# bark-simulator/planner-miqp

Measured on AMD Instinct MI355X. Metric: MIQP solves/sec to 1% gap, 2-agent x 20-step x 32-region, higher is better.
Workload: dtype f64

## Files before the change

include/miqp_gpu.h:

```cpp
#ifndef MIQP_GPU_H
#define MIQP_GPU_H

#include "miqp_types.h"

#ifdef __cplusplus
extern "C" {
#endif

typedef struct miqp_solver miqp_solver_t;

typedef struct miqp_solver_opts {
  int precision;
  int device;
  int nodes_per_round;
  int max_open_nodes;
  double gap_override;
  int verbose;
} miqp_solver_opts;

miqp_solver_t* miqp_solver_create(const miqp_solver_opts* opts);
void miqp_solver_destroy(miqp_solver_t* s);

int miqp_solver_set_params(miqp_solver_t* s, const miqp_model_params_c* p);

int miqp_solver_load_dat(miqp_solver_t* s, const char* path);

int miqp_solver_override_settings(miqp_solver_t* s, double max_solution_time, double relative_mip_gap_tolerance);

int miqp_solver_set_warmstart(miqp_solver_t* s, const miqp_raw_results_c* start, int warmstart_type);

int miqp_solver_solve(miqp_solver_t* s, double timestamp);

int miqp_solver_solve_batch(miqp_solver_t* const* solvers, int n, int* statuses);

int miqp_solver_solve_stream(miqp_solver_t* const* solvers, int n, int inflight, int* statuses);

int miqp_solver_solve_batch_multi(miqp_solver_t* const* solvers, int n, int gpus, int* statuses);

typedef int (*miqp_exchange_fn)(void* user, int op, void* buf, int count, int root);
int miqp_solver_solve_split(miqp_solver_t* s, double timestamp, int world, int rank, miqp_exchange_fn exchange, void* user);

int miqp_comm_unique_id(char* out128);
int miqp_comm_init(int world, int rank, const char* id128, int device);
int miqp_comm_finalize(void);
int miqp_solver_solve_split_rccl(miqp_solver_t* s, double timestamp);
int miqp_comm_selftest(miqp_exchange_fn exchange, void* user, int world, int rank);

int miqp_solver_split_roots(const miqp_solver_t* s, int world, int rank, int* root_of_pair, int* index, int* value, int cap, int* nroots_out, int* ncombos_out);

int miqp_solver_raw_sizes(const miqp_solver_t* s, int* out4);
int miqp_solver_lift_tables(const miqp_solver_t* s, double* out, int cap);

int miqp_solver_get_results(const miqp_solver_t* s, miqp_raw_results_c* out);

int miqp_solver_materialize_results(miqp_solver_t* const* solvers, int n, int threads);

int miqp_solver_get_properties(const miqp_solver_t* s, miqp_solution_properties_c* out);

int miqp_solver_get_dims(const miqp_solver_t* s, int* out6);

int miqp_solver_export_lp(const miqp_solver_t* s, const char* path);

int miqp_solver_write_dat(const miqp_solver_t* s, const char* path);

int miqp_solver_write_solution(const miqp_solver_t* s, const char* path);

int miqp_solver_write_mst(const miqp_solver_t* s, const char* path);

int miqp_solver_read_mst(miqp_solver_t* s, const char* path);

int miqp_solver_solve_fixed(miqp_solver_t* s, const miqp_raw_results_c* fixed, miqp_raw_results_c* out,
                            double* objective, int* iterations);

int miqp_solver_last_timing(const miqp_solver_t* s, double* out6);

int miqp_solver_last_active_set(const miqp_solver_t* s, double* out8);

int miqp_solver_last_fixed_route(const miqp_solver_t* s);

int miqp_solver_solve_fixed_batch(miqp_solver_t* s, const miqp_raw_results_c* const* fixed, int n, miqp_fixed_result_c* out, int* best);

int miqp_solver_fixed_batch_record(miqp_solver_t* s, int k, miqp_raw_results_c* out);

int miqp_gpu_fixed_result_size(void);
int miqp_gpu_fixed_batch_chunk(void);

int miqp_solver_set_pool(miqp_solver_t* s, int capacity);
int miqp_solver_pool_count(const miqp_solver_t* s);
int miqp_solver_pool_found(const miqp_solver_t* s, double* obj, int cap);
int miqp_solver_pool_solve(miqp_solver_t* s, miqp_fixed_result_c* out, int cap);
int miqp_solver_pool_record(miqp_solver_t* s, int k, miqp_raw_results_c* out);
int miqp_gpu_pool_max(void);

int miqp_solver_set_pool_filter(miqp_solver_t* s, int families);
int miqp_gpu_pool_signature(int cars, int steps, int obstacles, int families, const signed char* decisions, signed char* out, int len);
int miqp_solver_pool_signature(const miqp_solver_t* s, const miqp_raw_results_c* rec, int families, signed char* out, int cap);
int miqp_solver_pool_found_decisions(const miqp_solver_t* s, int k, signed char* out, int cap);

int miqp_solver_solve_fixed_multi(miqp_solver_t* const* solvers, int n, const miqp_raw_results_c* const* fixed, const int* first, miqp_fixed_result_c* out, int* best);
int miqp_solver_pool_solve_multi(miqp_solver_t* const* solvers, int n, miqp_fixed_result_c* out, int cap, int* counts);

int miqp_gpu_has_active_set(int num_cars, int num_steps);

int miqp_solver_launch_plan(const miqp_solver_t* s, int bc, int overlap, int par, const int* cls_n3, int cus, double free_gb, int flags, int* out, int cap);

int miqp_solver_last_setup(const miqp_solver_t* s, double* out3);

int miqp_solver_last_admission(const miqp_solver_t* s, double* out1);

const char* miqp_solver_last_error(const miqp_solver_t* s);


int miqp_fraction_parameters(int nr_regions, float max_velocity_fitting, double* out);
int miqp_fitting_polynomial_parameters(int nr_regions, float max_velocity_fitting, float min_velocity_fitting, double* out);
int miqp_mean_angles(const double* fraction_parameters, int nr_regions, double* out);
int miqp_limits_per_region(const double* fraction_parameters, int nr_regions, float long_min, float long_max, float lat_min, float lat_max,
                           double* min_x, double* max_x, double* min_y, double* max_y);
int miqp_calculate_region_idx(const double* fraction_parameters, int nr_regions, float vx, float vy, int* out);
int miqp_reserve_neighbor_regions(int* row, int nr_regions, int expansions);
int miqp_calculate_possible_regions(const double* fraction_parameters, int nr_regions, const double* theta_ref, int n, int* flags);
int miqp_reference_trajectory(const double* ref_xy, int n_ref, const double* state5, double dt, int num_points, double line_interp_inc, double vel_desired,
                              double delta_s_desired, double acc_lat_max, int vel_curve_dep, double* out);
int miqp_update_car(const double* settings12, const double* fraction_parameters, const double* initial_state6, const double* ref_xy, int n_ref, double desired_velocity,
                    double delta_s_desired, double timestep, int track_reference_positions, int is_ego, int num_cars, double* ref4N, int* possible_region, double* weights8);
int miqp_calculate_warmstart(const miqp_raw_results_c* last, miqp_raw_results_c* out, double ts, double minimum_region_change_speed);
int miqp_plan(miqp_solver_t* s, miqp_model_params_c* p, int* initial_region, int* possible_region, const miqp_raw_results_c* warmstart,
              int warmstart_type, double timestamp, int* status_out);

int miqp_initial_pose_check(const miqp_model_params_c* p);
int miqp_select_environment(const double* pieces_xy, const int* piece_off, int n_pieces, const double* traj_xy, const int* traj_off, int n_traj, int* selected);
int miqp_obstacle_intersects_environment(const double* pieces_xy, const int* piece_off, int n_pieces, const double* obstacle_xy, int n_steps, int is_static);
int miqp_bark_trajectory(const miqp_raw_results_c* results, int car, double start_time, double ts, double min_speed, double* out_rows5);
int miqp_obstacles_roi(double x, double y, double theta, double behind_distance, double front_distance, double side_distance, double* roi_xy);
int miqp_obstacle_intersects_environment_roi(const double* pieces_xy, const int* piece_off, int n_pieces, const double* obstacle_xy, int n_steps, int is_static, const double* roi_xy);
int miqp_environment_warmstart(const miqp_raw_results_c* last, miqp_raw_results_c* out, const int* ids_old, int n_old, const int* ids_new, int n_new);

int miqp_solver_certify(miqp_solver_t* s, const miqp_raw_results_c* candidate, miqp_certificate_c* out);
int miqp_solver_certify_batch(miqp_solver_t* const* solvers, int n, miqp_certificate_c* out);
int miqp_gpu_certificate_size(void);
int miqp_gpu_certify_last_timing(double* out4);

const char* miqp_gpu_version(void);

#ifdef __cplusplus
}
#endif
#endif
```

planner_miqp_amd/csrc/as_onchip.hip:

```cpp
namespace miqp {

#ifdef MIQP_PROFILE
#define ASP_T(var) const long long var = clock64()
#define ASP_ACC(k, t0, t1) asp_[k] += (unsigned long long)((t1) - (t0))
#else
#define ASP_T(var)
#define ASP_ACC(k, t0, t1)
#endif
constexpr int AS_MAXSTEP = 220;
constexpr double AS_VTOL = 1.0e-8;
constexpr double AS_DEP = 1.0e-8;
constexpr int AS_MT = 64;
constexpr int AS_MSTR = AS_MT * (AS_MT + 1) / 2;

__host__ __device__ constexpr bool as_shape_ok(int C, int N) { return (C == 1 || C == 2) && N >= 1 && N <= 2 * OC_NSL; }

template <int C> __device__ inline int as_col(int pq) { return C == 2 ? ((pq & 3) << 2) | (pq >> 2) : ((pq & 1) << 2) | (pq >> 1); }
template <int C> __device__ inline int as_pcol(int q) { return C == 2 ? ((q & 3) << 2) | (q >> 2) : ((q & 3) << 1) | (q >> 2); }
template <int C> struct AsDecode {
  static constexpr bool LANE_BOUNDS = true, ROW_IDENTITY = true, MARKS = true;
  static __device__ int col(int l) { return as_col<C>(oc_pcol<C, true>(l)); }
};

template <int C, int NSL, int GCAP = miqp::OC_GCAP>
__global__ void __launch_bounds__(64, (GCAP > 128 ? 1 : 2)) as_onchip_kernel(DevBuf B) {
  static_assert(C == 1 || C == 2, "a stage of 16 columns holds the chains of up to two cars");
  constexpr bool CM = true;
  constexpr bool BIG = GCAP > 128;
  constexpr int OC_GCAP = GCAP, OC_GSLOTS = OC_GCAP / 64, OC_GCOEF = oc_gcoef_of(OC_GCAP);
  constexpr int NX = 6 * C, NZ = 8 * C, NCH = 2 * C;
  const Layout& Y = B.Y;
  const int tid = threadIdx.x, lg = tid >> 4, lc = tid & 15;
  const int par = lg >> 1, side = lg & 1;
  const double bsgn = side ? -1.0 : 1.0;
  WAVE_DUMP(BIG ? 1 : 4);
  const int* const clist = BIG && B.cls_take ? B.cls_list + (size_t)(B.cls_take - 1) * B.batch_cap : nullptr;
  const int nbatch = clist ? (B.cls_count[B.cls_take - 1] < B.batch_cap ? B.cls_count[B.cls_take - 1] : B.batch_cap) : (*B.batch_count < B.batch_cap ? *B.batch_count : B.batch_cap);
  const int N = Y.N, NSLOT = Y.NSLOT;
  extern __shared__ double lds[];
  char* const L0 = (char*)lds;
  const OcLds LL = oc_lds_layout(N, Y.fixlen, OC_GCAP, !BIG);
  double* const Z = (double*)(L0 + LL.z);
  double* const scr = (double*)(L0 + LL.u);
  double* const V = (double*)(L0 + LL.u);
  unsigned long long* const bkey = (unsigned long long*)(L0 + LL.r);
  const int SPAN = LL.gmeta - LL.u;
  double* const kref = (double*)(L0 + LL.u + SPAN - N * 32);
  double* const kff = kref - N * 4;
  double* const KS = kff - N * 16;
  const int STG_CAP = (SPAN - N * 192) / 8;
  uint4* const gmeta = (uint4*)(L0 + LL.gmeta);
  double* const gcoef = (double*)(L0 + LL.gcoef);
  double* const grhs = (double*)(L0 + LL.grhs);
  double* const Wd = (double*)(L0 + LL.wd);
  int* const sstart = (int*)(L0 + LL.sstart);
  unsigned short* const cand = (unsigned short*)(L0 + LL.cand);
  signed char* const fix = (signed char*)(L0 + LL.fix);
  __shared__ int sh_node;
  __shared__ unsigned long long sh_stat[32];
  if (tid < 32) sh_stat[tid] = 0ull;
  const unsigned long long lt = (1ull << tid) - 1ull;

  const int chunk = B.as_chunk > 0 ? B.as_chunk : 1;
  int run_next = 0, run_end = 0;
  const int quota = BIG ? 0 : B.as_quota; int handed = 0;
#ifdef MIQP_PROFILE
  const unsigned long long wv_c0 = __builtin_amdgcn_s_memtime(), wv_r0 = __builtin_amdgcn_s_memrealtime();
  unsigned long long wv_first = 0; int wv_nodes = 0;
  if (!BIG && tid == 0) wv_first = atomicMin(&B.prof[120], wv_r0);
#endif
  for (;;) {
    __syncthreads();
    if (run_next >= run_end) {
      if (quota > 0 && handed >= quota) break;
      ++handed;
      if (tid == 0) sh_node = atomicAdd(B.work_counter, chunk);
      __syncthreads();
      run_next = __builtin_amdgcn_readfirstlane(sh_node); run_end = run_next + chunk;
      if (run_next >= nbatch) break;
    }
    const int slot_ = run_next++;
    if (slot_ >= nbatch) { run_next = run_end; continue; }
    const int node = clist ? __builtin_amdgcn_readfirstlane(clist[slot_]) : slot_;
    {
      const int cls = B.batch_large ? (int)B.batch_large[node] : (is_probe_word(B.batch_depth[node]) ? 1 : 0);
      if (cls != (BIG ? 1 : 0)) continue;
    }
    WAVE_DUMP_NODE();
    const int inst = __builtin_amdgcn_readfirstlane(B.batch_inst[node]);
    const double* D = B.inst_d + (size_t)inst * Y.dstride;
    const int* T = B.inst_i + (size_t)inst * Y.istride;
    const double ts = D[Y.d_glob + 7];
    const double aqs = 2.0 * D[Y.d_misc + 0];
    const double iaq = aqs > 0.0 ? 1.0 / aqs : 0.0;
    {
      const signed char* src = B.pool_fix + (size_t)B.batch_node[node] * Y.fixlen;
      for (int k = tid; k < Y.fixlen; k += 64) fix[k] = src[k];
      if (tid < 16) Wd[tid] = tid < NZ ? D[Y.d_wd + oc_lcol<C, CM>(as_pcol<C>(tid))] : 0.0;
      for (int k = tid; k < N * 32; k += 64) bkey[k] = ~0ull;
      for (int k = tid; k <= N + 1; k += 64) sstart[k] = 0;
    }
    __syncthreads();
    const double* Rf = D + Y.d_ref;
    double cutoff = 1e300;
    {
      const double inc0 = fmin(inc_from_key(*(volatile unsigned long long*)&B.inc_key[inst]), B.inc_ext[inst]);
      const double gap_ = is_probe_word(B.batch_depth[node]) ? 0.0 : B.inst_gap[inst];
      if (B.use_cutoff && inc0 < 1e300) cutoff = inc0 - gap_ * (1e-10 + fabs(inc0)) - B.inst_const[inst];
    }

#ifdef MIQP_PROFILE
    unsigned long long asp_[12] = {0, 0, 0, 0, 0, 0, 0, 0, 0, 0, 0, 0};
#endif
    ASP_T(ta0);
#define OC_DECODE_POLICY AsDecode<C>
#include "oc_decode_body.inc"
#undef OC_DECODE_POLICY
    if (overflow) {
      if (B.batch_A) B.batch_A[(size_t)node * 64 + tid] = 0xFFFFu;
      if (tid == 0) {
        if (B.ring_M) B.batch_Mtag[node] = 0ull;
        B.batch_ok[node] = 5; B.pool_big[B.batch_node[node]] |= (BIG ? 2 : 1); if (B.stats) { atomicAdd(&B.stats[3], 1ull); atomicAdd(&B.stats[8 + (ngen >= 512 ? 15 : ngen / 32)], 1ull); }
      }
      continue;
    }
    const int NM = sstart[N + 1];
    OC_WAVE_SYNC();

    ASP_T(ta1); ASP_ACC(0, ta0, ta1);
#ifdef MIQP_PROFILE
    asp_[9] += (unsigned long long)(ocd_t_sparse - ta0); asp_[11] += (unsigned long long)(ta1 - ocd_t_rows);
#endif
    double brhs[NSL];
    unsigned int bact = 0u, binA = 0u, ginA = 0u;
#pragma unroll
    for (int k = 0; k < NSL; ++k) {
      const int i = 2 * k + par;
      brhs[k] = 1e300;
      if (i < N && lc < NZ) {
        const unsigned long long key = bkey[(i * 2 + side) * 16 + lc];
        if (key != ~0ull) { brhs[k] = key2d(key); bact |= 1u << k; }
      }
    }
    OC_WAVE_SYNC();

    const double h1 = ts, h2 = 0.5 * ts * ts, h3 = ts * ts * ts / 6.0;
    const double* const tb = D + Y.d_astab;
    if constexpr (C == 2) {
      for (int k = tid; k < N * 16; k += 64) KS[k] = tb[k];
      for (int k = tid; k < N * 4; k += 64) kref[k] = tb[N * 16 + k];
    } else {
      for (int k = tid; k < N * 8; k += 64) KS[(k >> 3) * 16 + (k & 7)] = tb[k];
      for (int k = tid; k < N * 2; k += 64) kref[(k >> 1) * 4 + (k & 1)] = tb[N * 8 + k];
    }
    OC_WAVE_SYNC();
    typedef double d2_t __attribute__((ext_vector_type(2)));
    auto subst = [&](const bool fromx0, const int itop, const int iend, double* const out) {
      for (int k = tid; k < (N - 1) * 4; k += 64) if ((k >> 2) > itop) kff[k] = fromx0 ? kref[k] : 0.0;
      if (tid < NCH) {
        const int ch = tid;
        double p0 = 0.0, p1 = 0.0, p2 = 0.0;
        int i0 = itop;
        if (itop >= N - 1) { const d2_t a = *(const d2_t*)(V + (N - 1) * 16 + 4 * ch); p0 = a[0]; p1 = a[1]; p2 = V[(N - 1) * 16 + 4 * ch + 2]; i0 = N - 2; }
        if (i0 >= 0) {
          d2_t va = *(const d2_t*)(V + i0 * 16 + 4 * ch), vb = *(const d2_t*)(V + i0 * 16 + 4 * ch + 2);
          d2_t ka = *(const d2_t*)(KS + (i0 * 4 + ch) * 4), kb = *(const d2_t*)(KS + (i0 * 4 + ch) * 4 + 2);
          double kr = fromx0 ? kref[i0 * 4 + ch] : 0.0;
          for (int i = i0; i >= 0; --i) {
            const int j = i > 0 ? i - 1 : 0;
            const d2_t nva = *(const d2_t*)(V + j * 16 + 4 * ch), nvb = *(const d2_t*)(V + j * 16 + 4 * ch + 2);
            const d2_t nka = *(const d2_t*)(KS + (j * 4 + ch) * 4), nkb = *(const d2_t*)(KS + (j * 4 + ch) * 4 + 2);
            const double nkr = fromx0 ? kref[j * 4 + ch] : 0.0;
            const double su = vb[1] + h3 * p0 + h2 * p1 + h1 * p2;
            const double sx0 = va[0] + p0, sx1 = va[1] + h1 * p0 + p1, sx2 = vb[0] + h2 * p0 + h1 * p1 + p2;
            kff[i * 4 + ch] = fma(su, kb[1], kr);
            p0 = sx0 - ka[0] * su; p1 = sx1 - ka[1] * su; p2 = sx2 - kb[0] * su;
            va = nva; vb = nvb; ka = nka; kb = nkb; kr = nkr;
          }
        }
      }
      OC_WAVE_SYNC();
      if (tid < NCH) {
        const int ch = tid;
        double x0 = 0.0, x1 = 0.0, x2 = 0.0;
        if (fromx0) { const int c = ch >> 1, s = ch & 1; x0 = D[Y.d_x0 + 6 * c + 3 * s]; x1 = D[Y.d_x0 + 6 * c + 3 * s + 1]; x2 = D[Y.d_x0 + 6 * c + 3 * s + 2]; }
        const int ie = iend < N - 1 ? iend : N - 2;
        d2_t ka = *(const d2_t*)(KS + ch * 4), kb = *(const d2_t*)(KS + ch * 4 + 2);
        double kf = kff[ch];
        for (int i = 0; i <= ie; ++i) {
          const int j = i < N - 2 ? i + 1 : N - 2;
          const d2_t nka = *(const d2_t*)(KS + (j * 4 + ch) * 4), nkb = *(const d2_t*)(KS + (j * 4 + ch) * 4 + 2);
          const double nkf = kff[j * 4 + ch];
          const double u = -kf - (ka[0] * x0 + ka[1] * x1 + kb[0] * x2);
          d2_t oa, ob; oa[0] = x0; oa[1] = x1; ob[0] = x2; ob[1] = u;
          *(d2_t*)(out + i * 16 + 4 * ch) = oa; *(d2_t*)(out + i * 16 + 4 * ch + 2) = ob;
          const double n0 = x0 + h1 * x1 + h2 * x2 + h3 * u, n1 = x1 + h1 * x2 + h2 * u, n2 = x2 + h1 * u;
          x0 = n0; x1 = n1; x2 = n2;
          ka = nka; kb = nkb; kf = nkf;
        }
        if (iend >= N - 1 || ie == N - 2) { d2_t oa, ob; oa[0] = x0; oa[1] = x1; ob[0] = x2; ob[1] = 0.0; *(d2_t*)(out + (ie + 1) * 16 + 4 * ch) = oa; *(d2_t*)(out + (ie + 1) * 16 + 4 * ch + 2) = ob; }
      }
      OC_WAVE_SYNC();
    };
    auto row_dot = [&](int id, const double* vec) -> double {
      if (id < 1024) return (((id >> 4) & 1) ? -1.0 : 1.0) * vec[(id >> 5) * 16 + (id & 15)];
      const uint4 m4 = gmeta[id - 1024];
      const int off = (int)(m4.z & 0xFFFFu), nn = (int)((m4.z >> 16) & 7u), i = (int)((m4.z >> 20) & 0x7FFu);
      double a = 0.0;
#pragma unroll
      for (int k = 0; k < 6; ++k) if (k < nn) a += gcoef[off + k] * vec[i * 16 + ((m4.w >> (4 * k)) & 15u)];
      return a;
    };
    auto row_soft = [&](int id) -> bool { return id >= 1024 && (gmeta[id - 1024].z & 0x80000000u) != 0u; };
    auto zeroV = [&]() { for (int k = tid; k < N * 16; k += 64) V[k] = 0.0; OC_WAVE_SYNC(); };
    auto objective = [&]() -> double {
      double o = 0.0;
      for (int k = tid; k < N * 16; k += 64) { const int q = k & 15; if (q < NZ) { const double d = Z[k] - Rf[(k >> 4) * NZ + oc_lcol<C, CM>(as_pcol<C>(q))]; o += Wd[q] * d * d; } }
      return wave_sum(o);
    };

    int arow = -1, astage = -1; double alam = 0.0, arhs = 0.0;
    double M[64];
#pragma unroll
    for (int b = 0; b < 64; ++b) M[b] = 0.0;
    unsigned long long used = 0ull;
    auto rank1 = [&](const double u, const double alpha, const unsigned long long mask) {
#pragma unroll
      for (int g8 = 0; g8 < 8; ++g8) {
        if ((mask >> (8 * g8)) & 0xFFull) {
#pragma unroll
          for (int j = 0; j < 8; ++j) { const int b = 8 * g8 + j; M[b] = fma(u * readlane_d(u, b), alpha, M[b]); }
        }
      }
    };
    auto refresh = [&]() {
      zeroV();
      const double FX = 274877906944.0, IFX = 1.0 / 274877906944.0;
      if (arow >= 0 && alam != 0.0) {
        if (arow < 1024) atomicAdd((unsigned long long*)&V[(arow >> 5) * 16 + (arow & 15)], (unsigned long long)(long long)__double2ll_rn((((arow >> 4) & 1) ? -alam : alam) * FX));
        else {
          const uint4 m4 = gmeta[arow - 1024];
          const int off = (int)(m4.z & 0xFFFFu), nn = (int)((m4.z >> 16) & 7u), i = (int)((m4.z >> 20) & 0x7FFu);
#pragma unroll
          for (int k = 0; k < 6; ++k) if (k < nn) atomicAdd((unsigned long long*)&V[i * 16 + ((m4.w >> (4 * k)) & 15u)], (unsigned long long)(long long)__double2ll_rn(gcoef[off + k] * alam * FX));
        }
      }
      OC_WAVE_SYNC();
      for (int k = tid; k < N * 16; k += 64) V[k] = (double)(long long)__double_as_longlong(V[k]) * IFX;
      const int amax = (int)wave_max((double)astage);
      OC_WAVE_SYNC();
      subst(true, amax, N - 1, Z);
    };
    if constexpr (C == 2) { for (int k = tid; k < N * 16; k += 64) Z[k] = tb[N * 20 + k]; }
    else { for (int k = tid; k < N * 16; k += 64) Z[k] = (k & 15) < NZ ? tb[N * 10 + (k >> 4) * NZ + (k & 15)] : 0.0; }
    OC_WAVE_SYNC();
    ASP_T(ta2); ASP_ACC(1, ta1, ta2);
    int steps = 0, ndrop = 0, ok = 1, nwarm = 0, nfast = 0, ncold = 0;
    bool infeas = false, fail = false;
    int why = 0;
    if (B.pool_A && (B.batch_depth[node] >> 6) >= 1 && B.batch_node[node] < B.z_cap) {
      const int rec = B.batch_node[node];
      const unsigned int pa = B.pool_A[(size_t)rec * 64 + tid];
      int cid = -1;
      int ownl = 0;
      if (pa < 1024u) ownl = (int)((((pa >> 5) & 1u) * 2u + ((pa >> 4) & 1u)) << 4 | (pa & 15u));
      const unsigned int ob = (unsigned int)__shfl((int)bact, ownl);
      if (pa < 1024u) { if ((ob >> (pa >> 6)) & 1u) cid = (int)pa; }
      else if (pa != 0xFFFFu) {
        const int pc = (int)pa - 1024;
        int lo = 0, hi = NM;
        while (lo < hi) { const int mid = (lo + hi) >> 1; if ((int)cand[mid] < pc) lo = mid + 1; else hi = mid; }
        if (lo < NM && (int)cand[lo] == pc) cid = 1024 + lo;
      }
      const unsigned long long u0p = __ballot(pa != 0xFFFFu);
      const unsigned long long u0 = __ballot(cid >= 0);
      if (u0) {
        arow = cid;
        astage = cid < 0 ? -1 : (cid < 1024 ? (cid >> 5) : (int)((gmeta[cid - 1024].z >> 20) & 0x7FFu));
        int nmp = 0; unsigned long long moff = 0ull;
        if (B.ring_M) {
          const unsigned long long tg = B.pool_Mtag[rec];
          const unsigned long long c_ = tg >> 8;
          if (tg != 0ull && *(volatile unsigned long long*)B.ring_head - c_ < B.ring_doubles - B.ring_margin) { nmp = (int)(tg & 255ull); moff = c_ % B.ring_doubles; }
        }
// ... 161 lines not shown
        const int r = q * 64 + tid;
        if (r < NM && !((ginA >> q) & 1u)) { const double rh_ = grhs[r]; const double v = row_dot(1024 + r, Z) - rh_; if (v > bv) { bv = v; brh = rh_; bid = 1024 + r; } }
      }
      const double vmax = wave_max(bv);
      if (!(vmax > AS_VTOL)) break;
      if (steps >= AS_MAXSTEP || used == ~0ull || !(vmax < 1e290)) { fail = true; why = used == ~0ull ? 1 : 2; break; }
      const int src = __builtin_amdgcn_readfirstlane(__ffsll((long long)__ballot(bv == vmax)) - 1);
      const int pid = __builtin_amdgcn_readlane(bid, src);
      const bool psoft = row_soft(pid);
      const double prhs = readlane_d(brh, src);
      ASP_T(tb1); ASP_ACC(2, tb0, tb1);
      zeroV();
      if (pid < 1024) { if (tid == 0) V[(pid >> 5) * 16 + (pid & 15)] = ((pid >> 4) & 1) ? -1.0 : 1.0; }
      else {
        const uint4 m4 = gmeta[pid - 1024];
        const int off = (int)(m4.z & 0xFFFFu), nn = (int)((m4.z >> 16) & 7u), i = (int)((m4.z >> 20) & 0x7FFu);
        if (tid < nn) V[i * 16 + ((m4.w >> (4 * tid)) & 15u)] = gcoef[off + tid];
      }
      const int pstage = pid < 1024 ? (pid >> 5) : (int)((gmeta[pid - 1024].z >> 20) & 0x7FFu);
      const int amax_ = (int)wave_max((double)astage);
      OC_WAVE_SYNC();
      subst(false, pstage, amax_ > pstage ? amax_ : pstage, V);
      ASP_T(tb2); ASP_ACC(3, tb1, tb2);
      double q = arow >= 0 ? -row_dot(arow, V) : 0.0;
      const double Spp = -row_dot(pid, V) + (psoft ? iaq : 0.0);
      double vp = vmax, lp = 0.0;
      steps++;
      ASP_T(tb3); ASP_ACC(4, tb2, tb3);
      for (;;) {
        double r = 0.0;
#pragma unroll
        for (int g8 = 0; g8 < 8; ++g8) {
          if ((used >> (8 * g8)) & 0xFFull) {
#pragma unroll
            for (int j = 0; j < 8; ++j) { const int b = 8 * g8 + j; r = fma(M[b], readlane_d(q, b), r); }
          }
        }
        if (arow < 0) r = 0.0;
        const double curv = Spp - wave_sum(q * r);
        const double ratio = (arow >= 0 && r > 1e-13) ? alam / r : 1e300;
        const double td = wave_min(ratio);
        const int kd = td < 1e299 ? __builtin_amdgcn_readfirstlane(__ffsll((long long)__ballot(ratio == td)) - 1) : -1;
        if (!(curv == curv) || !(Spp > 0.0)) { fail = true; why = 3; break; }
        const bool dep = !(curv > AS_DEP * Spp);
        double t; bool full;
        if (dep) { if (kd < 0) { infeas = true; break; } t = td; full = false; }
        else { const double tp = vp / curv; if (tp <= td) { t = tp; full = true; } else { t = td; full = false; } }
        if (arow >= 0) { alam = fma(-t, r, alam); if (alam < 0.0) alam = 0.0; }
        lp += t;
        Dval += t * (vp - 0.5 * t * (dep ? 0.0 : curv));
        if (lp > RHO_EL) { infeas = true; break; }
        if (full) {
          const int s = __builtin_amdgcn_readfirstlane(__ffsll((long long)~used) - 1);
          double u = arow >= 0 ? r : 0.0;
          if (tid == s) u = -1.0;
          const unsigned long long nmask = used | (1ull << s);
          rank1(u, 1.0 / curv, nmask);
          if (tid == s) { arow = pid; alam = lp; astage = pstage; arhs = prhs; }
          used = nmask;
          if (pid < 1024) { if (tid == ((((pid >> 5) & 1) * 2 + ((pid >> 4) & 1)) << 4 | (pid & 15))) binA |= 1u << (pid >> 6); }
          else { const int rr_ = pid - 1024; if (tid == (rr_ & 63)) ginA |= 1u << (rr_ >> 6); }
          break;
        }
        vp -= t * (dep ? 0.0 : curv);
        const int idk = __builtin_amdgcn_readlane(arow, kd);
        if (idk < 1024) { if (tid == ((((idk >> 5) & 1) * 2 + ((idk >> 4) & 1)) << 4 | (idk & 15))) binA &= ~(1u << (idk >> 6)); }
        else { const int rr_ = idk - 1024; if (tid == (rr_ & 63)) ginA &= ~(1u << (rr_ >> 6)); }
        double m = 0.0;
#pragma unroll
        for (int b = 0; b < 64; ++b) m = (b == kd) ? M[b] : m;
        const double mkk = readlane_d(m, kd);
        if (!(mkk > 0.0)) { fail = true; why = 4; break; }
        rank1(m, -1.0 / mkk, used);
#pragma unroll
        for (int b = 0; b < 64; ++b) if (b == kd || tid == kd) M[b] = 0.0;
        if (tid == kd) { arow = -1; astage = -1; alam = 0.0; q = 0.0; }
        used &= ~(1ull << kd);
        ndrop++; steps++;
        if (steps >= AS_MAXSTEP) { fail = true; why = 2; break; }
      }
      ASP_T(tb4); ASP_ACC(5, tb3, tb4);
      if (infeas || fail) break;
      refresh();
      ASP_T(tb5); ASP_ACC(6, tb4, tb5);
      if (Dval - 1e-9 * fabs(Dval) > cutoff + 1e-9 * fabs(cutoff)) { ok = 2; break; }
    }
    ASP_T(tc0);
    double viol = 0.0, scost = 0.0, lres = 0.0;
    if (!fail && !infeas && ok == 1) {
#pragma unroll
      for (int k = 0; k < NSL; ++k) { const int i = 2 * k + par; if ((bact >> k) & 1u) viol = fmax(viol, bsgn * Z[i * 16 + lc] - brhs[k]); }
#pragma unroll
      for (int q = 0; q < OC_GSLOTS; ++q) { const int r = q * 64 + tid; if (r < NM && !(gmeta[r].z & 0x80000000u)) viol = fmax(viol, row_dot(1024 + r, Z) - grhs[r]); }
      if (arow >= 0) {
        const bool sf = arow >= 1024 && row_soft(arow);
        const double res = row_dot(arow, Z) - arhs - (sf ? alam * iaq : 0.0);
        if (sf) { scost = 0.5 * alam * alam * iaq; viol = fmax(viol, res); }
        lres = alam * res;
      }
      viol = wave_max(viol); scost = wave_sum(scost);
      lres = fabs(wave_sum(lres));
    } else if (infeas) viol = 1.0;
    if (!fail && !infeas && ok == 1 && !(viol <= 5.0e-7)) { fail = true; why = 5; }
    if (BIG && infeas && B.as_probe_first && B.pump_max > 0 && is_probe_word(B.batch_depth[node]) && (cutoff > 1e299 || B.pump_inc)) fail = true;
    if (fail) {
      if (B.batch_A) B.batch_A[(size_t)node * 64 + tid] = 0xFFFFu;
      if (B.ring_M && tid == 0) B.batch_Mtag[node] = 0ull;
      if (tid == 0) { B.batch_ok[node] = 5; B.pool_big[B.batch_node[node]] |= 4; if (B.as_stats) { sh_stat[2] += 1ull; sh_stat[10 + (why < 6 ? why : 5)] += 1ull; } }
      continue;
    }
    const double obj = (infeas || ok == 2) ? Dval : objective() + scost;
    double* Zo = B.batch_Z + (size_t)node * N * NZ;
    for (int k = tid; k < N * 16; k += 64) { const int q = k & 15; if (q < NZ) Zo[(k >> 4) * NZ + oc_lcol<C, CM>(as_pcol<C>(q))] = Z[k]; }
    if (B.batch_A) {
      unsigned short enc = 0xFFFFu;
      if (!fail && !infeas && ok == 1 && arow >= 0) enc = arow < 1024 ? (unsigned short)arow : (unsigned short)(1024 + (int)cand[arow - 1024]);
      B.batch_A[(size_t)node * 64 + tid] = enc;
    }
    if (B.ring_M) {
      const int n_ = __popcll(used);
      unsigned long long tg_ = 0ull;
      OC_WAVE_SYNC();
      if (!fail && !infeas && ok == 1 && n_ >= 1 && n_ <= AS_MT && n_ * (n_ + 1) * 4 <= LL.total) {
        double* const stg = (double*)L0;
        const int ra = __popcll(used & lt);
#pragma unroll
        for (int b8 = 0; b8 < 64; ++b8) {
          if ((used >> b8) & 1ull) {
            const int rb = __popcll(used & ((1ull << b8) - 1ull));
            if (arow >= 0 && ra >= rb) stg[ra * (ra + 1) / 2 + rb] = M[b8];
          }
        }
        const int len = n_ * (n_ + 1) / 2;
        unsigned long long cnt_ = 0ull;
        if (tid == 0) cnt_ = atomicAdd(B.ring_head, (unsigned long long)len);
        cnt_ = ((unsigned long long)(unsigned int)__builtin_amdgcn_readfirstlane((int)(cnt_ >> 32)) << 32) | (unsigned int)__builtin_amdgcn_readfirstlane((int)cnt_);
        tg_ = (cnt_ << 8) | (unsigned long long)n_;
        OC_WAVE_SYNC();
        const unsigned long long o_ = cnt_ % B.ring_doubles, rd_ = B.ring_doubles;
        for (int k = tid; k < len; k += 64) { unsigned long long q_ = o_ + (unsigned long long)k; if (q_ >= rd_) q_ -= rd_; B.ring_M[q_] = stg[k]; }
      }
      if (tid == 0) B.batch_Mtag[node] = tg_;
    }
    if (tid == 0) {
      B.batch_obj[node] = obj; B.batch_viol[node] = viol; B.batch_ok[node] = ok;
      B.batch_bound[node] = lres + 1e-9 * (1.0 + fabs(obj));
      B.batch_it[node] = steps;
      atomicAdd((unsigned long long*)&B.inst_nodes[inst], 1ull);
      atomicAdd((unsigned long long*)&B.inst_iters[inst], (unsigned long long)steps);
#ifdef MIQP_PROFILE
      ++wv_nodes;
      { const long long tc1 = clock64(); asp_[7] += (unsigned long long)(tc1 - tc0);
        for (int q_ = 0; q_ < 9; ++q_) atomicAdd(&B.prof[80 + q_], asp_[q_]);
        atomicAdd(&B.prof[92], asp_[9]); atomicAdd(&B.prof[93], asp_[11]);
        atomicAdd(&B.prof[90], 1ull); atomicAdd(&B.prof[91], (unsigned long long)steps); }
#endif
      if (B.as_stats) {
        sh_stat[0] += 1ull; sh_stat[1] += (unsigned long long)steps; sh_stat[3] += (unsigned long long)ndrop;
        sh_stat[4] += infeas ? 1ull : 0ull; sh_stat[5] += ok == 2 ? 1ull : 0ull; sh_stat[6] += (unsigned long long)__popcll(used); sh_stat[7] += (unsigned long long)nwarm; sh_stat[8] += (unsigned long long)nfast; sh_stat[9] += (unsigned long long)ncold;
        if (BIG) { const int og_ = B.pool_origin ? (int)B.pool_origin[B.batch_node[node]] : 0; sh_stat[20] += 1ull; sh_stat[21] += (unsigned long long)steps; if (og_ == 14) { sh_stat[22] += 1ull; sh_stat[23] += (unsigned long long)steps; }
          sh_stat[24 + (ngen <= 64 ? 0 : ngen <= 96 ? 1 : ngen <= 128 ? 2 : ngen <= 192 ? 3 : 4)] += 1ull; if (is_probe_word(B.batch_depth[node]) && og_ != 14) sh_stat[29] += 1ull; }
      }
    }
  }
  __syncthreads();
  if (B.as_stats && tid < 32 && sh_stat[tid] != 0ull) atomicAdd(&B.as_stats[tid], sh_stat[tid]);
#ifdef MIQP_PROFILE
  if (!BIG && tid == 0) {
    const unsigned long long wv_c1 = __builtin_amdgcn_s_memtime(), wv_r1 = __builtin_amdgcn_s_memrealtime();
    atomicAdd(&B.prof[94], wv_c1 - wv_c0); atomicAdd(&B.prof[95], wv_r1 - wv_r0); atomicAdd(&B.prof[96], 1ull);
    atomicMin(&B.prof[122], wv_r1); atomicMax(&B.prof[121], wv_r1);
    const unsigned long long dl = wv_r0 > wv_first ? wv_r0 - wv_first : 0ull;
    const int hb = dl < 5000 ? 0 : dl < 20000 ? 1 : dl < 50000 ? 2 : dl < 100000 ? 3 : dl < 200000 ? 4 : dl < 400000 ? 5 : dl < 800000 ? 6 : 7;
    atomicAdd(&B.prof[128 + hb], 1ull);
    const int nb = wv_nodes == 0 ? 0 : wv_nodes <= 4 ? 1 : wv_nodes <= 16 ? 2 : wv_nodes <= 32 ? 3 : wv_nodes <= 64 ? 4 : 5;
    atomicAdd(&B.prof[136 + nb], 1ull);
    if (B.prof[125] == 300 && blockIdx.x < 4096) {
      unsigned int hw, xcc;
      asm volatile("s_getreg_b32 %0, hwreg(HW_REG_HW_ID)" : "=s"(hw));
      asm volatile("s_getreg_b32 %0, hwreg(HW_REG_XCC_ID)" : "=s"(xcc));
      unsigned long long* const w = B.prof + 160 + 4 * blockIdx.x;
      w[0] = wv_r0; w[1] = wv_r1; w[2] = ((unsigned long long)xcc << 32) | hw; w[3] = (unsigned long long)wv_nodes;
    }
  }
#endif
}

}
```

planner_miqp_amd/csrc/ipm_onchip.hip:

```cpp
#ifndef MIQP_PHI_BRANCH
#define MIQP_PHI_BRANCH 1
#endif
namespace miqp {

constexpr int OC_GSLOTS = OC_GCAP / 64;
#ifndef MIQP_OC_PF
#define MIQP_OC_PF 4
#endif
constexpr int OC_PF = MIQP_OC_PF;
#ifndef MIQP_OC_GRP
#define MIQP_OC_GRP 5
#endif
constexpr int OC_GRP = MIQP_OC_GRP;
constexpr int OC_NSL = 10;

#ifdef MIQP_PROFILE
#define OCP_T(var) const long long var = clock64()
#define OCP_ACC(k, t0, t1) ocp_[k] += (unsigned long long)((t1) - (t0))
#elif defined(MIQP_ISA_MARKS)
#define OCP_T(var) asm volatile("; OCMARK " #var)
#define OCP_ACC(k, t0, t1)
#else
#define OCP_T(var)
#define OCP_ACC(k, t0, t1)
#endif
__host__ __device__ inline int oc_gain_doubles(int N) { return N * 64; }

template <int C, bool CM> __device__ inline int oc_pcol(int l) { return (CM && l < 6 * C) ? 2 * C * (l % 3) + l / 3 : l; }
template <int C, bool CM> __device__ inline int oc_lcol(int p) { return (CM && p < 6 * C) ? 3 * (p % (2 * C)) + p / (2 * C) : p; }
template <int C, bool CM> struct IpmDecode {
  static constexpr bool LANE_BOUNDS = false, ROW_IDENTITY = false, MARKS = false;
  static __device__ int col(int l) { return oc_pcol<C, CM>(l); }
};
template <int CTRL> __device__ inline double dpp_shift0(double x) {
  int lo = __double2loint(x), hi = __double2hiint(x);
  lo = __builtin_amdgcn_update_dpp(0, lo, CTRL, 0xF, 0xF, true);
  hi = __builtin_amdgcn_update_dpp(0, hi, CTRL, 0xF, 0xF, true);
  return __hiloint2double(hi, lo);
}

__device__ inline int fresh_lane() {
  int l;
  asm volatile("v_mbcnt_lo_u32_b32 %0, -1, 0\n\tv_mbcnt_hi_u32_b32 %0, -1, %0" : "=v"(l));
  return l;
}

__device__ inline void row_weight(double s, double lam, double t, bool soft, double aq, double tau, double& w, double& lk) {
  const double il = frcp(lam);
  double zz, r2mu = 0.0;
  if (!soft) { const double mu = RHO_EL - lam, im = frcp(mu); zz = t * im; r2mu = (tau - t * mu) * im; }
  else zz = frcp(aq);
  w = frcp(s * il + zz);
  lk = lam + ((tau - s * lam) * il - r2mu) * w;
}

template <int C, int NSL, int ABL = 0, int GCAP = miqp::OC_GCAP>
__global__ void __launch_bounds__(64, (GCAP > 128 ? 1 : 2)) ipm_onchip_kernel(DevBuf B) {
  constexpr int OC_ABL = ABL;
  constexpr int OC_GCAP = GCAP, OC_GSLOTS = GCAP / 64, OC_GCOEF = oc_gcoef_of(GCAP);
  constexpr bool BIG = GCAP > 128;
  static_assert(GCAP % 64 == 0 && GCAP <= 512, "general rows: whole register slots per lane, flags of up to 8 slots");
  constexpr bool CM = C == 2 && !(ABL & 1024);
  static_assert(C <= 2, "one 16 x 16 tile per stage");
  constexpr int NX = 6 * C, NU = 2 * C, NZ = 8 * C;
  constexpr int KB = (NX + 3) / 4;
  constexpr int RU = NX / 4, GU0 = NX % 4;
  const Layout& Y = B.Y;
  const int tid = threadIdx.x, lg = tid >> 4, lc = tid & 15;
  const int par = lg >> 1, side = lg & 1;
  const double bsgn = side ? -1.0 : 1.0;
  WAVE_DUMP(2);
  const int* const clist = BIG && B.cls_take ? B.cls_list + (size_t)(B.cls_take - 1) * B.batch_cap : nullptr;
  const int nbatch = clist ? (B.cls_count[B.cls_take - 1] < B.batch_cap ? B.cls_count[B.cls_take - 1] : B.batch_cap) : BIG && B.ovf_mode == 1 ? *B.ovf_count : (*B.batch_count < B.batch_cap ? *B.batch_count : B.batch_cap);
  const int N = Y.N, NSLOT = Y.NSLOT;
  extern __shared__ double lds[];
  char* const L0 = (char*)lds;
  const OcLds LL = oc_lds_layout(N, Y.fixlen, GCAP);
  double* const Z = (double*)(L0 + LL.z);
  double* const Dg = (double*)(L0 + LL.u);
  double* const Gd = Dg + N * 16;
  double* const dZ = Dg;
  double* const scr = Dg;
  unsigned long long* const bkey = (unsigned long long*)(L0 + LL.r);
  double* const gswfs = (double*)(L0 + LL.r);
#ifndef MIQP_KL0_PACK
#define MIQP_KL0_PACK 1
#endif
  constexpr int GS = (CM && MIQP_KL0_PACK) ? 1 : 2;
  constexpr int KL0N = OC_KL0 + (GS == 1 ? OC_GCAP / 64 : 0);
  double* const KL0 = gswfs + GS * OC_GCAP;
  uint4* const gmeta = (uint4*)(L0 + LL.gmeta);
  double* const gcoef = (double*)(L0 + LL.gcoef);
  double* const grhs = (double*)(L0 + LL.grhs);
  double* const Wd = (double*)(L0 + LL.wd);
  int* const sstart = (int*)(L0 + LL.sstart);
  unsigned short* const cand = (unsigned short*)(L0 + LL.cand);
  signed char* const fix = (signed char*)(L0 + LL.fix);
  double* const KG = B.kgain + (size_t)blockIdx.x * oc_gain_doubles(N);
  const double* KGs;
  { const unsigned long long a = (unsigned long long)KG;
    KGs = (const double*)(((unsigned long long)(unsigned int)__builtin_amdgcn_readfirstlane((int)(a >> 32)) << 32) | (unsigned int)__builtin_amdgcn_readfirstlane((int)a)); }
  const bool gown = lg < NU && lc <= NX;
  __shared__ int sh_node;
  const unsigned long long lt = (1ull << tid) - 1ull;

  for (;;) {
    __syncthreads();
    if (tid == 0) sh_node = atomicAdd(B.work_counter, 1);
    __syncthreads();
    if (__builtin_amdgcn_readfirstlane(sh_node) >= nbatch) break;
    const int node = __builtin_amdgcn_readfirstlane(clist ? clist[sh_node] : BIG && B.ovf_mode == 1 ? B.ovf_list[sh_node] : sh_node);
    if ((BIG && B.ovf_mode == 2) || (!BIG && B.skip_probes)) {
      const bool marked = B.batch_large ? B.batch_large[node] != 0 : is_probe_word(B.batch_depth[node]);
      if (BIG ? !marked : marked) continue;
      if (BIG && B.as_split && B.batch_large[node] != 2) continue;
    }
    WAVE_DUMP_NODE();
    const int inst = __builtin_amdgcn_readfirstlane(B.batch_inst[node]);
    const double* D = B.inst_d + (size_t)inst * Y.dstride;
    const int* T = B.inst_i + (size_t)inst * Y.istride;
    const double ts = D[Y.d_glob + 7];
    const double aqs = 2.0 * D[Y.d_misc + 0];
    {
      const signed char* src = B.pool_fix + (size_t)B.batch_node[node] * Y.fixlen;
      for (int k = tid; k < Y.fixlen; k += 64) fix[k] = src[k];
      if (tid < 16) Wd[tid] = tid < NZ ? D[Y.d_wd + oc_lcol<C, CM>(tid)] : 0.0;
      for (int k = tid; k < N * 16; k += 64) Z[k] = 0.0;
      for (int k = tid; k < N * 32; k += 64) bkey[k] = ~0ull;
      for (int k = tid; k <= N + 1; k += 64) sstart[k] = 0;
    }
    const bool warm = B.ws_on == 2 || (B.ws_on && B.pool_Z && (B.batch_depth[node] >> 6) >= 1 && B.batch_node[node] < B.z_cap);
    __syncthreads();
    if (warm) {
      const double* zp = B.ws_on == 2 ? B.inc_Z + (size_t)inst * N * NZ : B.pool_Z + (size_t)B.batch_node[node] * N * NZ;
      for (int k = tid; k < N * 16; k += 64) { const int q = k & 15; if (q < NZ) Z[k] = zp[(k >> 4) * NZ + oc_lcol<C, CM>(q)]; }
      OC_WAVE_SYNC();
    } else {
    if (tid < NX) Z[tid] = D[Y.d_x0 + oc_lcol<C, CM>(tid)];
    OC_WAVE_SYNC();
    for (int i = 0; i + 1 < N; ++i) {
      if (tid < NX) {
        double acc = 0;
        if (CM) { const int k = tid / (2 * C); acc = Z[i * 16 + tid]; if (k < 2) acc += ts * Z[i * 16 + tid + 2 * C]; if (k < 1) acc += 0.5 * ts * ts * Z[i * 16 + tid + 4 * C]; }
        else for (int q = 3 * (tid / 3); q < 3 * (tid / 3) + 3; ++q) acc += ab_entry<C>(tid, q, ts) * Z[i * 16 + q];
        Z[(i + 1) * 16 + tid] = acc;
      }
      OC_WAVE_SYNC();
    }
    }
    const double* Rf = D + Y.d_ref;
    const double cutoff = node_cutoff(B, inst, node);
#ifdef MIQP_PROFILE
    unsigned long long ocp_[12] = {0, 0, 0, 0, 0, 0, 0, 0, 0, 0, 0, 0};
#endif
    OCP_T(tp_d0);
    double abr[KB];
#pragma unroll
    for (int kb = 0; kb < KB; ++kb) abr[kb] = (!CM && 4 * kb + lg < NX && lc < NZ) ? ab_entry<C>(4 * kb + lg, lc, ts) : 0.0;

#define OC_DECODE_POLICY IpmDecode<C, CM>
#include "oc_decode_body.inc"
#undef OC_DECODE_POLICY
    if (overflow && !BIG && B.bounce) {
      if (tid == 0) { B.batch_ok[node] = 5; B.pool_big[B.batch_node[node]] |= 1; if (B.stats) { atomicAdd(&B.stats[3], 1ull); atomicAdd(&B.stats[8 + (ngen >= 512 ? 15 : ngen / 32)], 1ull); } }
      continue;
    }
    if (overflow && BIG && B.as_split) {
      if (tid == 0) { B.batch_ok[node] = 5; B.pool_big[B.batch_node[node]] |= 2; }
      continue;
    }
    if (overflow) {
      if (tid == 0) { const int q = atomicAdd(BIG ? B.ovf2_count : B.ovf_count, 1); (BIG ? B.ovf2_list : B.ovf_list)[q] = node; if (B.stats && !BIG) { atomicAdd(&B.stats[3], 1ull); atomicAdd(&B.stats[8 + (ngen >= 512 ? 15 : ngen / 32)], 1ull); if (ngen >= 480) { atomicMax(&B.stats[5], (unsigned long long)ngen); atomicAdd(&B.stats[6], (unsigned long long)ngen); atomicAdd(&B.stats[7], 1ull); } } }
      continue;
    }
    const int NM = sstart[N + 1];
    OC_WAVE_SYNC();
    if (tid == 0) { int a = 0; for (int i = 0; i <= N; ++i) { const int n = sstart[i]; a += n; sstart[i] = a; } }
    OC_WAVE_SYNC();

    double bs[NSL], bl[NSL], bt[NSL];
    unsigned int bact = 0u;
    double csum = 0.0, tsum = 0.0; int cnt = 0;
#pragma unroll
    for (int k = 0; k < NSL; ++k) {
// ... 527 lines not shown
```

planner_miqp_amd/csrc/miqp_gpu.hip:

```cpp
#include <hip/hip_runtime.h>
#include <dlfcn.h>

#include <algorithm>
#include <chrono>
#include <cmath>
#include <cstdio>
#include <cstdlib>
#include <cstring>
#include <map>
#include <memory>
#include <atomic>
#include <mutex>
#include <string>
#include <thread>
#include <vector>

#include "../../include/miqp_gpu.h"
#include "kernels.hip"
#include "wire_formats.hpp"
#include "planner_core.hpp"
#include "lp_export.hpp"

__attribute__((constructor)) static void miqp_gpu_hw_queues() { setenv("GPU_MAX_HW_QUEUES", "8", 0); }

// ... 1272 lines not shown
}
bool take_polished(const DevCtx& X, miqp_solver_t* const* S, int n, const HostTables& H, const Polished& P, Results& R) {
  const DevBuf& B = X.B; const Layout& Y = X.Y;
  std::vector<double> h_pZ((size_t)n * Y.N * Y.nz);
  HIP_OK(hipMemcpy(h_pZ.data(), B.batch_Z, h_pZ.size() * 8, hipMemcpyDeviceToHost));
  for (int k = 0; k < n; ++k) {
    if (!(R.inc[k] < 1e299)) continue;
    if (P.viol[k] <= FEAS_TOL && (P.ok[k] || P.it[k] >= 10)) {
      int nign = 0; for (int q = 0; q < Y.C * Y.O * Y.N * 5; ++q) nign += R.fix[(size_t)k * Y.fixlen + Y.f_obs + q] >= Y.L;
      R.inc[k] = P.obj[k] + H.h_const[k] + nign * S[k]->inst.w_slack_obs;
      std::copy(h_pZ.begin() + (size_t)k * Y.N * Y.nz, h_pZ.begin() + (size_t)(k + 1) * Y.N * Y.nz, R.Z.begin() + (size_t)k * Y.N * Y.nz);
    }
  }
  return true;
}

bool split_broadcast(const SplitCtx* split, const SplitState& sp, Results& R) {
  std::vector<unsigned char> buf(8 + R.Z.size() * 8 + R.fix.size());
  unsigned long long w[2] = {R.inc[0] < 1e299 ? ((host_d2key(R.inc[0]) & ~0xFFFFFull) | (unsigned long long)split->rank) : ~0ull, ~0ull};
  if (split->fn(split->user, 0, w, 2, 0) != 0) { std::fprintf(stderr, "[miqp_gpu] incumbent exchange failed\n"); return false; }
  if (w[0] < 0xFFF0000000000000ull) {
    const int owner = (int)(w[0] & 0xFFFFFull);
    if (owner == split->rank) { std::memcpy(buf.data(), &R.inc[0], 8); std::memcpy(buf.data() + 8, R.Z.data(), R.Z.size() * 8); std::memcpy(buf.data() + 8 + R.Z.size() * 8, R.fix.data(), R.fix.size()); }
    if (split->fn(split->user, 1, buf.data(), (int)buf.size(), owner) != 0) { std::fprintf(stderr, "[miqp_gpu] solution broadcast failed\n"); return false; }
    std::memcpy(&R.inc[0], buf.data(), 8); std::memcpy(R.Z.data(), buf.data() + 8, R.Z.size() * 8); std::memcpy(R.fix.data(), buf.data() + 8 + R.Z.size() * 8, R.fix.size());
    R.lb[0] = std::min(sp.lb, R.inc[0]);
  }
  R.flags[0] = sp.finished ? 0 : 1; R.oc[0] = 0; R.dn[0] = 1;
  return true;
}

struct CallTimes { double t_setup = 0, t_ctx = 0, t_tables = 0, t_solve = 0, ms_ipm = 0, ms_std = 0; float ms_all = 0; bool ctx_built = false, std_timed = false; };

void report(miqp_solver_t* const* S, int* statuses, const Layout& Y, const HostTables& H, const Rounds& L, const Results& R, const CallTimes& T, bool split) {
  const int n = L.n;
  long long tot_iters = 0; for (int k = 0; k < n; ++k) tot_iters += R.iters[k];
  for (int k = 0; k < n; ++k) {
    miqp_solver* s = S[k];
    bool have = R.inc[k] < 1e299;
    bool unfinished = (R.flags[k] & 3) || R.oc[k] > 0 || !R.dn[k];
    if (!split && k >= L.next_q && !H.h_done[k]) {
      s->status = MIQP_STATUS_FAILED_SEG_FAULT; s->has_sol = false; s->props.objective = NAN; s->props.gap = NAN; s->props.best_bound = NAN; s->props.status = 0; s->props.time = 0.0;
      s->err = "the queue was abandoned before this instance was admitted";
      statuses[k] = s->status; continue;
    }
    s->props.time = L.t_done[k] >= 0 ? L.t_done[k] : std::max(0.0, T.t_solve - L.t_admit[k]);
    s->admit_s = L.t_admit[k];
    s->props.NrIterations = (int)std::min<long long>(R.iters[k], 2147483647LL); s->props.nodes = R.nodes[k];
    s->props.NrSolutionPool = R.ninc[k];
    s->timing[0] = T.ms_all * 1e-3; s->timing[1] = T.ms_ipm * 1e-3; s->timing[2] = (double)(L.nev / 2); s->timing[3] = (double)L.launched_nodes;
    s->timing[4] = (double)tot_iters; s->timing[5] = (double)R.rowiters;
    s->as_timing[0] = (double)R.as[0]; s->as_timing[1] = (double)R.as[1]; s->as_timing[2] = (double)R.as[2]; s->as_timing[3] = (double)R.as[3];
    s->as_timing[4] = (double)R.as[6]; s->as_timing[5] = (double)R.as[7]; s->as_timing[6] = T.ms_std * 1e-3; s->as_timing[7] = T.std_timed ? (double)(L.nev / 2) : 0.0;
    s->setup[0] = T.t_setup; s->setup[1] = T.t_ctx; s->setup[2] = T.ctx_built ? 1.0 : 0.0;
    s->err.clear();
    if (L.stalled[k] && unfinished) s->err = "retired without a proof: no progress for 64 branch-and-bound rounds (not a time-limit verdict)";
    if (have) {
      s->status = MIQP_STATUS_SUCCESS; s->has_sol = true;
      s->props.objective = R.inc[k];
      double lb = std::min(R.lb[k], R.inc[k]);
      const double lb_tol = R.inc[k] - H.h_gap[k] * std::fabs(R.inc[k]);
      lb = std::min(lb, lb_tol);
      s->props.best_bound = lb; s->props.gap = std::fabs(lb - R.inc[k]) / (1e-10 + std::fabs(R.inc[k]));
      if (lb == lb_tol && s->props.gap > H.h_gap[k]) s->props.gap = H.h_gap[k];
      s->props.status = unfinished ? MIQP_CPX_STAT_TIME_LIM_FEAS : (s->props.gap <= 1e-9 ? MIQP_CPX_STAT_OPTIMAL : MIQP_CPX_STAT_OPTIMAL_TOL);
      s->Z.assign(R.Z.begin() + (size_t)k * Y.N * Y.nz, R.Z.begin() + (size_t)(k + 1) * Y.N * Y.nz);
      s->comp.assign(R.fix.begin() + (size_t)k * Y.fixlen, R.fix.begin() + (size_t)(k + 1) * Y.fixlen);
    } else {
      s->status = unfinished ? (L.stalled[k] ? MIQP_STATUS_FAILED_SEG_FAULT : MIQP_STATUS_FAILED_TIMEOUT) : MIQP_STATUS_FAILED_NO_SOLUT;
      s->props.objective = NAN; s->props.gap = NAN; s->props.best_bound = R.lb[k];
      s->props.status = unfinished ? MIQP_CPX_STAT_TIME_LIM_INFEAS : MIQP_CPX_STAT_INFEASIBLE;
    }
    statuses[k] = s->status;
  }
  if (L.abandoned) std::fprintf(stderr, "[miqp_gpu] the round loop was abandoned with %d of %d instances never admitted: they report FAILED_SEG_FAULT, the call fails\n", n - L.next_q, n);
}

bool pool_prepare(DevCtx& X, miqp_solver_t* const* S, int n);
bool pool_read_back(const DevCtx& X, miqp_solver_t* const* S, int n, const Results& R);

bool solve_batch_impl(miqp_solver_t* const* S, int n, int* statuses, const SplitCtx* split = nullptr, int inflight = 0, int lane = 0, int lanes = 1) {
  for (int k = 0; k < n; ++k) { statuses[k] = MIQP_STATUS_FAILED_SEG_FAULT; if (S[k]) { S[k]->status = MIQP_STATUS_FAILED_SEG_FAULT; S[k]->has_sol = false; S[k]->rescache.reset(); S[k]->drop_pool(); } }
  if (split && n != 1) return false;
  BatchShape bs = batch_layout(S, n);
  if (!bs.ok) { for (int k = 0; k < n; ++k) { if (S[k]) S[k]->err = bs.err; statuses[k] = MIQP_STATUS_FAILED_SEG_FAULT; } std::fprintf(stderr, "[miqp_gpu] %s\n", bs.err.c_str()); return false; }
  const Layout& Y = bs.Y;
  const miqp_solver_opts& O0 = S[0]->opts;
  auto fail_all = [&](const char* why) { if (why) std::fprintf(stderr, "[miqp_gpu] %s\n", why); for (int k = 0; k < n; ++k) statuses[k] = MIQP_STATUS_FAILED_SEG_FAULT; return false; };
  for (int k = 1; k < n; ++k) if (S[k]->opts.device != O0.device) return fail_all("instances of one batch must name the same device (use miqp_solver_solve_batch_multi to span devices)");
  const double t_enter = wall_s();
  DevCtx* Xp = ctx_for_device(O0.device, lane);
  if (!Xp) return fail_all(nullptr);
  warn_ignored_switches();
  DevCtx& X = *Xp;
  std::lock_guard<std::mutex> ctx_lock(X.mu);
  if (hipSetDevice(X.device) != hipSuccess) return fail_all("hipSetDevice failed");
  const CallSwitches sw = read_call_switches();
  const CallShape sh = plan_call(Y, O0, n, inflight, lanes, split != nullptr, sw);
  const size_t l_ipm = ipm_lds_bytes(Y), l_eval = eval_lds_bytes(Y, sw.seq_kinds);
  CallTimes T;
  {
    bool setup_ok = ctx_prepare(X, Y, n, sh.NS, sh.open_cap, sh.npr, sh.MAXR, sh.clamp_open, lanes, &T.ctx_built);
    if (setup_ok && (l_ipm > 160 * 1024 || l_eval > 160 * 1024)) { std::fprintf(stderr, "[miqp_gpu] instance too large for LDS (%zu bytes)\n", l_ipm); setup_ok = false; }
    if (setup_ok && !set_kernel_lds(Y, l_ipm, l_eval)) setup_ok = false;
    if (setup_ok && !pool_prepare(X, S, n)) setup_ok = false;
    if (split) {
      unsigned long long w = setup_ok ? 1ull : 0ull;
      if (split->fn(split->user, 0, &w, 1, 0) != 0) return fail_all("set-up exchange failed");
      if (setup_ok && w == 0ull) return fail_all("another rank of the tree split failed its set-up");
    }
    if (!setup_ok) return fail_all(nullptr);
  }
  T.t_ctx = wall_s() - t_enter;
  HostTables H;
  prepare_instances(S, Y, sh, split, H);
  T.t_tables = wall_s() - t_enter - T.t_ctx;
  apply_call_switches(X, sh, sw, H.h_gap);
  if (!upload_and_reset(X, H, sh)) return fail_all(nullptr);

  Rounds L(X, sh, H, split, O0.verbose, l_eval);
  if (!L.run()) return fail_all(nullptr);
  T.t_setup = L.t0 - t_enter;
  if (sw.dump_open && !dump_open_list(X, sw.dump_open, L.rounds, sh.NS, H.h_const[0])) return fail_all(nullptr);

  Polished P;
  if (!polish(X, n, P, T.ms_all)) return fail_all(nullptr);
#ifdef MIQP_PROFILE
  if (!print_profile(X)) return fail_all(nullptr);
#endif
  if (X.B.stats && !print_stats(X)) return fail_all(nullptr);
  if (process_switches().round_log) { std::fprintf(stderr, "[rounds]"); for (int v : L.round_bc) std::fprintf(stderr, " %d", v); std::fprintf(stderr, "\n"); }
  for (size_t e = 0; e + 1 < L.nev; e += 2) { float ms = 0; HIP_OK(hipEventElapsedTime(&ms, X.ipm_ev[e], X.ipm_ev[e + 1])); T.ms_ipm += ms; }
  T.std_timed = L.use_par;
  if (T.std_timed) for (size_t e = 0; e + 1 < L.nev; e += 2) { float ms = 0; if (hipEventElapsedTime(&ms, X.ipm_ev[e], X.std_ev[e / 2]) == hipSuccess) T.ms_std += ms; }
  T.t_solve = wall_s() - L.t0;

  Results R;
  if (!read_back(X, n, R) || !take_polished(X, S, n, H, P, R)) return fail_all(nullptr);
  if (X.pool.on && !pool_read_back(X, S, n, R)) return fail_all(nullptr);
  if (split && !split_broadcast(split, L.sp, R)) return fail_all(nullptr);
  report(S, statuses, Y, H, L, R, T, split != nullptr);
  for (int k = 0; k < n; ++k) if (!S[k]->has_sol) S[k]->drop_pool();
  if (sw.stats) std::fprintf(stderr, "[miqp_gpu stats] reachable-set diameter (L1) of instance 0: %.1f\n", H.D[Y.d_misc + 2]);
  if (sw.stats) std::fprintf(stderr, "[miqp_gpu stats] host: setup %.3f s (device context %.3f, instance tables and presolve %.3f, upload %.3f), rounds %.3f s (%d), results %.3f s\n", T.t_setup, T.t_ctx, T.t_tables, T.t_setup - T.t_ctx - T.t_tables, T.t_solve, L.rounds, wall_s() - L.t0 - T.t_solve);
  return !L.abandoned;
}

}

#include "certify.hip"
#include "fixed_batch.hip"
#include "solution_pool.hip"
#include "fixed_multi.hip"

extern "C" {

const char* miqp_gpu_version(void) { return "miqp_gpu 0.1 (gfx950)"; }

miqp_solver_t* miqp_solver_create(const miqp_solver_opts* opts) {
  miqp_solver* s = new miqp_solver();
  if (opts) s->opts = *opts; else { s->opts.precision = 12; s->opts.device = -1; s->opts.gap_override = -1; }
  if (s->opts.precision <= 0) s->opts.precision = 12;
  return s;
}

void miqp_solver_destroy(miqp_solver_t* s) { delete s; }

int miqp_solver_set_params(miqp_solver_t* s, const miqp_model_params_c* p) {
  if (!s || !p) return -1;
  s->has_inst = inst_from_params(p, s->opts.precision - 2, s->inst, s->err);
  s->rescache.reset(); s->drop_fixed_batch(); s->drop_pool();
  s->has_sol = false;
  if (!s->has_inst) std::fprintf(stderr, "[miqp_gpu] %s\n", s->err.c_str());
  return s->has_inst ? 0 : -2;
}

int miqp_solver_load_dat(miqp_solver_t* s, const char* path) {
  if (!s || !path) return -1;
  s->has_inst = inst_from_dat(path, s->inst, s->err);
  s->has_sol = false; s->rescache.reset(); s->drop_fixed_batch(); s->drop_pool();
  if (!s->has_inst) std::fprintf(stderr, "[miqp_gpu] %s\n", s->err.c_str());
  return s->has_inst ? 0 : -2;
}

int miqp_solver_override_settings(miqp_solver_t* s, double max_solution_time, double relative_mip_gap_tolerance) {
  if (!s || !s->has_inst) return -1;
  s->inst.tilim = max_solution_time; s->inst.gap = relative_mip_gap_tolerance;
  return 0;
}

int miqp_solver_get_dims(const miqp_solver_t* s, int* o) {
  if (!s || !s->has_inst) return -1;
  o[0] = s->inst.C; o[1] = s->inst.N; o[2] = s->inst.R; o[3] = s->inst.E; o[4] = s->inst.O; o[5] = s->inst.L;
  return 0;
}

int miqp_solver_set_warmstart(miqp_solver_t* s, const miqp_raw_results_c* start, int warmstart_type) {
  if (!s) return -1;
  if (warmstart_type == MIQP_WARMSTART_NONE || !start) { s->ws[0].reset(); s->ws[1].reset(); return 0; }
  const int slot = warmstart_type == MIQP_WARMSTART_LAST_SOLUTION ? 1 : 0;
  if (start->N < 2 || start->NrCars < 1 || start->NrRegions < 1 || start->NrEnvironments < 0 || start->NrObstacles < 0 || start->MaxLinesObstacles < 0 ||
      start->NrCarToCarCollisions != start->NrCars - 1) return -2;
  if (s->has_inst && !dims_match(*start, s->inst)) { s->ws[slot].reset(); return -3; }
  s->ws[slot].reset(new OwnedResults(start->NrCars, start->N, start->NrRegions, start->NrEnvironments, start->NrObstacles, start->MaxLinesObstacles));
  s->ws[slot]->copy_from(*start);
  return 0;
}

int miqp_solver_solve_batch(miqp_solver_t* const* solvers, int n, int* statuses) {
  if (!solvers || n < 1 || !statuses) return -1;
  return solve_batch_impl(solvers, n, statuses) ? 0 : -2;
}

int miqp_solver_solve_stream(miqp_solver_t* const* solvers, int n, int inflight, int* statuses) {
  if (!solvers || n < 1 || !statuses) return -1;
  int lanes = knob_int(KNOB_P("MIQP_LANES"), 1);
  if (lanes > 8) lanes = 8;
  while (lanes > 1 && (inflight <= 0 || inflight >= n || inflight / lanes < 128)) lanes--;
  if (lanes <= 1) return solve_batch_impl(solvers, n, statuses, nullptr, inflight) ? 0 : -2;
  for (int b = 0; b < n; ++b) { if (!solvers[b]) return -1; if (solvers[b]->opts.device != solvers[0]->opts.device) lanes = 1; }
  if (lanes <= 1) return solve_batch_impl(solvers, n, statuses, nullptr, inflight) ? 0 : -2;
  std::vector<std::vector<miqp_solver_t*>> sub(lanes); std::vector<std::vector<int>> st(lanes);
  for (int b = 0; b < n; ++b) sub[b % lanes].push_back(solvers[b]);
  std::vector<char> ok(lanes, 0);
  std::vector<std::thread> th;
  for (int l = 0; l < lanes; ++l) {
    st[l].assign(sub[l].size(), MIQP_STATUS_FAILED_SEG_FAULT);
    const int infl = (inflight + lanes - 1 - l) / lanes;
    th.emplace_back([&, l, infl] { ok[l] = solve_batch_impl(sub[l].data(), (int)sub[l].size(), st[l].data(), nullptr, infl, l, lanes) ? 1 : 0; });
  }
  for (auto& t : th) t.join();
  int rc = 0;
  for (int b = 0; b < n; ++b) statuses[b] = st[b % lanes][b / lanes];
  for (int l = 0; l < lanes; ++l) if (!ok[l]) rc = -2;
  return rc;
}

int miqp_solver_solve_batch_multi(miqp_solver_t* const* solvers, int n, int gpus, int* statuses) {
  if (!solvers || n < 1 || !statuses) return -1;
  int ndev = 0;
  if (hipGetDeviceCount(&ndev) != hipSuccess || ndev < 1) { std::fprintf(stderr, "[miqp_gpu] no HIP device: the solver has no CPU path\n"); for (int k = 0; k < n; ++k) statuses[k] = MIQP_STATUS_FAILED_SEG_FAULT; return -2; }
  if (gpus <= 0 || gpus > ndev) gpus = ndev;
  if (gpus > n) gpus = n;
  std::vector<std::vector<miqp_solver_t*>> shard(gpus); std::vector<std::vector<int>> st(gpus);
  for (int b = 0; b < n; ++b) { if (!solvers[b]) return -1; solvers[b]->opts.device = b % gpus; shard[b % gpus].push_back(solvers[b]); }
  std::vector<char> ok(gpus, 0);
  std::vector<std::thread> th;
  for (int g = 0; g < gpus; ++g) {
    st[g].assign(shard[g].size(), MIQP_STATUS_FAILED_SEG_FAULT);
    th.emplace_back([&, g] { ok[g] = solve_batch_impl(shard[g].data(), (int)shard[g].size(), st[g].data()) ? 1 : 0; });
  }
  for (auto& t : th) t.join();
  int rc = 0;
  for (int b = 0; b < n; ++b) statuses[b] = st[b % gpus][b / gpus];
  for (int g = 0; g < gpus; ++g) if (!ok[g]) rc = -2;
  return rc;
}

int miqp_solver_solve_split(miqp_solver_t* s, double timestamp, int world, int rank, miqp_exchange_fn exchange, void* user) {
  (void)timestamp;
  if (!s || !s->has_inst || world < 1 || rank < 0 || rank >= world || !exchange) return MIQP_STATUS_FAILED_SEG_FAULT;
  SplitCtx sc{world, rank, exchange, user};
  miqp_solver_t* one[1] = {s}; int st = MIQP_STATUS_FAILED_SEG_FAULT;
  if (!solve_batch_impl(one, 1, &st, &sc)) return MIQP_STATUS_FAILED_SEG_FAULT;
  return st;
}

int miqp_solver_split_roots(const miqp_solver_t* s, int world, int rank, int* root_of_pair, int* index, int* value, int cap, int* nroots_out, int* ncombos_out) {
  if (!s || !s->has_inst || world < 1 || rank < 0 || rank >= world) return -1;
  miqp_solver_t* one[1] = {const_cast<miqp_solver_t*>(s)};
  BatchShape bs = batch_layout(one, 1);
  if (!bs.ok) return -2;
  std::vector<double> D(bs.Y.dstride); std::vector<int> T(bs.Y.istride);
  compile_instance(s->inst, bs.Y, D.data(), T.data());
  std::vector<std::vector<std::pair<int, int>>> combos; split_roots(bs.Y, T.data(), combos, world);
  int np = 0, nr = 0;
  for (size_t q = 0; q < combos.size(); ++q) {
    if ((int)(q % (size_t)world) != rank) continue;
    for (auto& d : combos[q]) { if (np < cap) { if (root_of_pair) root_of_pair[np] = nr; if (index) index[np] = d.first; if (value) value[np] = d.second; } np++; }
    nr++;
  }
  if (nroots_out) *nroots_out = nr;
  if (ncombos_out) *ncombos_out = (int)combos.size();
  return np;
}

struct Id128 { char b[128]; };
namespace {
struct Rccl {
  void* lib = nullptr; void* comm = nullptr; int world = 0, rank = 0, device = -1; void* dbuf = nullptr; size_t dcap = 0; hipStream_t stream = nullptr;
  int (*GetUniqueId)(void*) = nullptr;
  int (*CommInitRank)(void**, int, Id128, int) = nullptr;
  int (*CommDestroy)(void*) = nullptr;
  int (*AllReduce)(const void*, void*, size_t, int, int, void*, hipStream_t) = nullptr;
  int (*Broadcast)(const void*, void*, size_t, int, int, void*, hipStream_t) = nullptr;
};
Rccl g_rccl; std::mutex g_rccl_mu;
bool rccl_load() {
  if (g_rccl.lib) return true;
  for (const char* nm : {"librccl.so.1", "librccl.so", "/opt/rocm/lib/librccl.so.1"}) { g_rccl.lib = dlopen(nm, RTLD_NOW | RTLD_LOCAL); if (g_rccl.lib) break; }
  if (!g_rccl.lib) { std::fprintf(stderr, "[miqp_gpu] librccl not found: %s\n", dlerror()); return false; }
  g_rccl.GetUniqueId = (int (*)(void*))dlsym(g_rccl.lib, "ncclGetUniqueId");
  g_rccl.CommInitRank = (int (*)(void**, int, Id128, int))dlsym(g_rccl.lib, "ncclCommInitRank");
  g_rccl.CommDestroy = (int (*)(void*))dlsym(g_rccl.lib, "ncclCommDestroy");
  g_rccl.AllReduce = (int (*)(const void*, void*, size_t, int, int, void*, hipStream_t))dlsym(g_rccl.lib, "ncclAllReduce");
  g_rccl.Broadcast = (int (*)(const void*, void*, size_t, int, int, void*, hipStream_t))dlsym(g_rccl.lib, "ncclBroadcast");
// ... 388 lines not shown
```

planner_miqp_amd/csrc/oc_decode.hip:

```cpp
namespace miqp {

constexpr int OC_GCAP = 128;
constexpr int OC_SCR = 32;
constexpr int OC_SSTR = 17;
constexpr int OC_KL0 = 6;

struct OcLds { int z, u, r, gmeta, gcoef, grhs, wd, sstart, cand, fix, total; };
constexpr int OC_GCAP_BIG = 320;
__host__ __device__ constexpr int oc_gcoef_of(int gcap) { return gcap == 128 ? 432 : gcap * 7 / 2; }
__host__ __device__ inline OcLds oc_lds_layout(int N, int fixlen, int OC_GCAP = miqp::OC_GCAP, bool as_std = false) {
  const int OC_GCOEF = oc_gcoef_of(OC_GCAP);
  OcLds L; int o = 0;
  L.z = o; o += N * 16 * 8;
  L.u = o; { int a = as_std ? N * 16 * 8 : N * 32 * 8, b = OC_SCR * OC_SSTR * 8; o += a > b ? a : b; }
  L.r = o; { int a = N * 32 * 8, b = as_std ? 0 : OC_GCAP * 16 + OC_KL0 * 64 * 8; o += a > b ? a : b; }
  L.gmeta = o; o += OC_GCAP * 16;
  L.gcoef = o; o += OC_GCOEF * 8;
  L.grhs = o; o += OC_GCAP * 8;
  L.wd = o; o += 16 * 8;
  L.sstart = o; o += ((N + 2) * 4 + 7) & ~7;
  L.cand = o; o += (OC_GCAP + 64) * 2;
  L.fix = o; o += (fixlen + 15) & ~15;
  L.total = (o + 15) & ~15;
  return L;
}

#define OC_WAVE_SYNC() do { __builtin_amdgcn_fence(__ATOMIC_RELEASE, "wavefront"); __builtin_amdgcn_wave_barrier(); __builtin_amdgcn_fence(__ATOMIC_ACQUIRE, "wavefront"); } while (0)

template <int C>
__device__ inline bool box_of_slot(const Layout& Y, const double* D, const int* T, const signed char* fix, int i, int slot, int& col, double& sgn, double& rhs) {
  if (slot >= C * Y.SC) return false;
  const int N = Y.N;
  const double* G = D + Y.d_glob;
  const int c = slot / Y.SC, rr = slot - c * Y.SC;
  const int code = i >= 1 ? (int)fix[Y.f_reg + c * N + i] : -1;
  const double* rt = code >= 0 ? D + Y.d_reg + (c * Y.P + (code >> 2)) * REGSZ : nullptr;
  if (rr < 7) {
    const double* Hc = (rt || rr < 3) ? D : region_hull(Y, D, T, fix, c, i);
    switch (rr) {
      case 0: col = 6 * c + 1; sgn = -1; rhs = -G[0]; break;
      case 1: col = 6 * c + 4; sgn = -1; rhs = -G[0]; break;
      case 2: col = 6 * c + 1; sgn = 1; rhs = G[1]; break;
      case 3: col = 6 * c + 2; sgn = 1; rhs = rt ? rt[12] : Hc[1]; break;
      case 4: col = 6 * c + 2; sgn = -1; rhs = -(rt ? rt[11] : Hc[0]); break;
      case 5: col = 6 * c + 5; sgn = 1; rhs = rt ? rt[14] : Hc[3]; break;
      default: col = 6 * c + 5; sgn = -1; rhs = -(rt ? rt[13] : Hc[2]); break;
    }
    return true;
  }
  if (rr < 11) {
    const int s = (rr - 7) >> 1; const bool up = ((rr - 7) & 1) == 0;
    double lo, hi;
    if (i == 0) { lo = D[Y.d_u0box + c * 4 + 2 * s]; hi = D[Y.d_u0box + c * 4 + 2 * s + 1]; }
    else if (rt) { lo = rt[15 + 2 * s]; hi = rt[16 + 2 * s]; }
    else { const double* Hc = region_hull(Y, D, T, fix, c, i); lo = Hc[4 + 2 * s]; hi = Hc[5 + 2 * s]; }
    col = 6 * C + 2 * c + s; sgn = up ? 1.0 : -1.0; rhs = up ? hi : -lo;
    return true;
  }
  if (rr < 16) {
    if (code < 0) return false;
    const int h = code & 3, k = rr - 11;
    if (h == 3) { col = 6 * c + (k < 2 ? 1 : 4); sgn = (k & 1) ? -1.0 : 1.0; rhs = G[6]; return true; }
    if (k == 2) {
      const int* hs = T + Y.i_hs + ((c * Y.P + (code >> 2)) * 2 + h) * 2;
      col = 6 * c + (hs[0] == 0 ? 1 : 4); sgn = -(double)hs[1]; rhs = -G[6];
      return true;
    }
    return false;
  }
  int q = rr - 16;
  const double* ed;
  if (q < 5 * Y.EL) {
    const int pt = q / Y.EL, k = q - pt * Y.EL;
    if (pt != 0) return false;
    const int e = Y.E == 1 ? 0 : (int)fix[Y.f_env + (c * N + i) * 5];
    ed = D + Y.d_env + (e * Y.EL + k) * 3;
  } else {
    q -= 5 * Y.EL;
    const int o = q / 5, pt = q - o * 5;
    if (pt != 0) return false;
    const int kk = (int)fix[Y.f_obs + ((c * Y.O + o) * N + i) * 5];
    ed = D + Y.d_obs + ((o * N + i) * Y.L + kk) * 3;
  }
  if (ed[1] == 0.0 && fabs(ed[0]) == 1.0) { col = 6 * c; sgn = ed[0]; rhs = ed[2]; return true; }
  if (ed[0] == 0.0 && fabs(ed[1]) == 1.0) { col = 6 * c + 3; sgn = ed[1]; rhs = ed[2]; return true; }
  return false;
}

template <int C>
__device__ inline bool slot_maybe(const Layout& Y, const signed char* fix, int i, int slot) {
  const int N = Y.N;
  if (slot < C * Y.SC) {
    const int c = slot / Y.SC, rr = slot - c * Y.SC;
    if (rr < 11) return true;
    if (i < 1) return false;
    const int code = (int)fix[Y.f_reg + c * N + i];
    if (rr < 16) return code >= 0 ? ((code & 3) != 3 || rr - 11 <= 3) : rr - 11 <= 1;
    int q = rr - 16;
    if (q < 5 * Y.EL) {
      if (Y.E < 1) return false;
      const int pt = q / Y.EL;
      const int e = Y.E == 1 ? 0 : (int)fix[Y.f_env + (c * N + i) * 5 + pt];
      return e >= 0 && (pt == 0 || code >= 0);
    }
    q -= 5 * Y.EL;
    const int o = q / 5, pt = q - o * 5;
    const int kk = (int)fix[Y.f_obs + ((c * Y.O + o) * N + i) * 5 + pt];
    return kk >= 0 && kk < Y.L && (pt == 0 || code >= 0);
  }
  if (C < 2 || i < 1) return false;
  const int q = slot - C * Y.SC;
  if (q < Y.NP * 8) { const int p = q >> 3, grp = (q & 7) >> 1; return (int)fix[Y.f_c2c + (p * N + i) * 4 + grp] >= 0; }
  const int q2 = q - Y.NP * 8, p = q2 >> 4, grp = (q2 >> 2) & 3, alt = q2 & 3;
  const int m = (int)fix[Y.f_c2n + (p * N + i) * 4 + grp];
  return m > 0 && ((m >> alt) & 1);
}

}
```

planner_miqp_amd/csrc/oc_decode_body.inc:

```
#ifdef MIQP_PROFILE
    long long ocd_t_sparse = 0, ocd_t_rows = 0;
#endif
    int ngen = 0;
    {
      unsigned long long* const bmp = (unsigned long long*)scr;
      const int nw = (N * NSLOT + 63) >> 6;
      unsigned short* const pre = (unsigned short*)(bmp + nw);
      for (int k = tid; k < nw; k += 64) bmp[k] = 0ull;
      OC_WAVE_SYNC();
      const int cls_off[8] = {0, 7, 11, 16, 16 + Y.EL, 16 + 5 * Y.EL, C * Y.SC, C * Y.SC + 8 * Y.NP};
      const int cls_cnt[8] = {7, 4, 5, Y.EL, 4 * Y.EL, 5 * Y.O, 8 * Y.NP, 16 * Y.NP};
      auto take = [&](int i, int slot) {
        if (decode_row<C, false>(Y, D, T, fix, i, slot, nullptr).active) {
          int col; double sg, rh;
          if (box_of_slot<C>(Y, D, T, fix, i, slot, col, sg, rh)) atomicMin(&bkey[(i * 2 + (sg < 0.0 ? 1 : 0)) * 16 + OC_DECODE_POLICY::col(col)], d2key(rh));
          else { const int pcode = i * NSLOT + slot; atomicOr(&bmp[pcode >> 6], 1ull << (pcode & 63)); }
        }
      };
      unsigned short* const plist = pre + ((nw + 1 + 3) & ~3);
      const int LCAP = (int)(((char*)(L0 + LL.r) - (char*)plist) / 2) - 64;
      int nlist = 0;
      auto flush = [&]() {
        OC_WAVE_SYNC();
        for (int j0 = 0; j0 < nlist; j0 += 64) if (j0 + tid < nlist) { const int pc = plist[j0 + tid]; const int i = pc / NSLOT; take(i, pc - i * NSLOT); }
        OC_WAVE_SYNC();
        nlist = 0;
      };
      if constexpr (OC_DECODE_POLICY::LANE_BOUNDS) {
        for (int e0 = 0; e0 < C * N; e0 += 64) {
          const int e = e0 + tid;
          if (e < C * N) {
            const int c = e / N, i = e - c * N;
            const double* G = D + Y.d_glob;
            const int code = i >= 1 ? (int)fix[Y.f_reg + c * N + i] : -1;
            const unsigned int skip = i >= 1 ? (unsigned int)T[Y.i_boxskip + c * N + i] : 0x7Fu;
            const double* rt = code >= 0 ? D + Y.d_reg + (c * Y.P + (code >> 2)) * REGSZ : nullptr;
            const double* Hc = (!rt && i >= 1) ? region_hull(Y, D, T, fix, c, i) : nullptr;
            auto put = [&](int col, bool neg, double rh) { atomicMin(&bkey[(i * 2 + (neg ? 1 : 0)) * 16 + OC_DECODE_POLICY::col(col)], d2key(rh)); };
            if (i >= 1) {
              const double a_lo_x = rt ? rt[11] : Hc[0], a_hi_x = rt ? rt[12] : Hc[1], a_lo_y = rt ? rt[13] : Hc[2], a_hi_y = rt ? rt[14] : Hc[3];
              if (!(skip & 1u)) put(6 * c + 1, true, -G[0]);
              if (!(skip & 2u)) put(6 * c + 4, true, -G[0]);
              if (!(skip & 4u)) put(6 * c + 1, false, G[1]);
              if (!(skip & 8u)) put(6 * c + 2, false, a_hi_x);
              if (!(skip & 16u)) put(6 * c + 2, true, -a_lo_x);
              if (!(skip & 32u)) put(6 * c + 5, false, a_hi_y);
              if (!(skip & 64u)) put(6 * c + 5, true, -a_lo_y);
            }
            if (i <= N - 2) {
#pragma unroll
              for (int s_ = 0; s_ < 2; ++s_) {
                double lo, hi;
                if (i == 0) { lo = D[Y.d_u0box + c * 4 + 2 * s_]; hi = D[Y.d_u0box + c * 4 + 2 * s_ + 1]; }
                else if (rt) { lo = rt[15 + 2 * s_]; hi = rt[16 + 2 * s_]; }
                else { lo = Hc[4 + 2 * s_]; hi = Hc[5 + 2 * s_]; }
                put(6 * C + 2 * c + s_, false, hi); put(6 * C + 2 * c + s_, true, -lo);
              }
            }
          }
        }
      }
#pragma unroll 1
      for (int cl = 0; cl < 8; ++cl) {
#ifdef MIQP_PROFILE
        if (OC_DECODE_POLICY::MARKS && cl == 2) ocd_t_sparse = clock64();
#endif
        const int cnt = cls_cnt[cl], off = cls_off[cl];
        const bool percar = cl < 6;
        const int per = percar ? C * cnt : cnt, total = N * per;
        for (int e0 = 0; e0 < total; e0 += 64) {
          const int e = e0 + tid;
          int i = 0, slot = 0; bool in = e < total;
          if (in) { i = e / per; const int rem = e - i * per; slot = percar ? (rem / cnt) * Y.SC + off + rem % cnt : off + rem; }
          if (cl < 2) {
            if constexpr (!OC_DECODE_POLICY::LANE_BOUNDS) { if (in) take(i, slot); }
            continue;
          }
          const bool cnd = in && slot_maybe<C>(Y, fix, i, slot);
          const unsigned long long mk = __ballot(cnd);
          if (cnd) plist[nlist + __popcll(mk & lt)] = (unsigned short)(i * NSLOT + slot);
          nlist += __popcll(mk);
          if (nlist > LCAP) flush();
        }
      }
      flush();
      if (tid == 0) { int a = 0; for (int k = 0; k < nw; ++k) { pre[k] = (unsigned short)(a < 65535 ? a : 65535); a += __popcll(bmp[k]); } pre[nw] = (unsigned short)(a < 65535 ? a : 65535); }
      OC_WAVE_SYNC();
      ngen = pre[nw];
      if (ngen <= OC_GCAP)
        for (int k = tid; k < nw; k += 64) {
          unsigned long long bits = bmp[k]; int pos = pre[k];
          while (bits) { const int b = __ffsll((long long)bits) - 1; cand[pos++] = (unsigned short)(k * 64 + b); bits &= bits - 1ull; }
        }
      OC_WAVE_SYNC();
    }
#ifdef MIQP_PROFILE
    if (OC_DECODE_POLICY::MARKS) ocd_t_rows = clock64();
#endif
    bool overflow = ngen > OC_GCAP;
    int ncoef = 0;
    for (int c0 = 0; c0 < ngen && !overflow; c0 += OC_SCR) {
      double* g = scr + (tid & (OC_SCR - 1)) * OC_SSTR;
      RowOut r; r.active = false; r.rhs = 0; r.aq = 0;
      int i = 0, nn = 0;
      const bool mine = tid < OC_SCR && c0 + tid < ngen;
      int slot_ = 0;
      if (mine) { const int pcode = cand[c0 + tid]; i = pcode / NSLOT; slot_ = pcode - i * NSLOT; r = decode_row<C, true>(Y, D, T, fix, i, slot_, g); }
      unsigned long long map = 0ull; unsigned int cols = 0u;
      double v6[6];
#pragma unroll
      for (int k = 0; k < 6; ++k) v6[k] = 0.0;
      if (mine) {
        for (int q = 0; q < NZ; ++q) {
          const double v = g[q];
          if (v != 0.0 && nn < 6) {
#pragma unroll
            for (int k = 0; k < 6; ++k) if (k == nn) v6[k] = v;
            const int pq = OC_DECODE_POLICY::col(q);
            map |= (unsigned long long)(nn + 1) << (4 * pq); cols |= (unsigned int)pq << (4 * nn); nn++;
          }
        }
      }
      const bool keep = mine && nn > 0;
      const unsigned long long mk = __ballot(keep);
      const unsigned long long b0 = __ballot(keep && (nn & 1)), b1 = __ballot(keep && (nn & 2)), b2 = __ballot(keep && (nn & 4));
      const int tot = __popcll(b0) + 2 * __popcll(b1) + 4 * __popcll(b2);
      if (ncoef + tot > OC_GCOEF) { overflow = true; break; }
      if (keep) {
        const int idx = sstart[N + 1] + __popcll(mk & lt);
        const int off = ncoef + __popcll(b0 & lt) + 2 * __popcll(b1 & lt) + 4 * __popcll(b2 & lt);
#pragma unroll
        for (int k = 0; k < 6; ++k) if (k < nn) gcoef[off + k] = v6[k];
        uint4 m4; m4.x = (unsigned int)map; m4.y = (unsigned int)(map >> 32);
        m4.z = (unsigned int)off | ((unsigned int)nn << 16) | ((unsigned int)i << 20) | (r.aq > 0.0 ? 0x80000000u : 0u); m4.w = cols;
        gmeta[idx] = m4; grhs[idx] = r.rhs;
        if constexpr (OC_DECODE_POLICY::ROW_IDENTITY) cand[idx] = (unsigned short)(i * NSLOT + slot_);
        else atomicAdd(&sstart[i + 1], 1);
      }
      OC_WAVE_SYNC();
      if (tid == 0) sstart[N + 1] += __popcll(mk);
      ncoef += tot;
      OC_WAVE_SYNC();
    }
```

planner_miqp_amd/csrc/solve_diag.hpp:

```cpp
#pragma once

inline void debug_sync(hipStream_t st, int round, const char* stage, int nodes = -1) {
  hipError_t e_ = hipStreamSynchronize(st);
  if (nodes >= 0) std::fprintf(stderr, "[dbg] round %d %s (%d nodes): %s\n", round, stage, nodes, hipGetErrorString(e_));
  else std::fprintf(stderr, "[dbg] round %d %s: %s\n", round, stage, hipGetErrorString(e_));
}

inline bool trace_selection(const DevCtx& X, int rounds, int bc) {
  const DevBuf& B = X.B;
  std::vector<double> sb(bc); std::vector<int> sd(bc); double io_ = 0; int md_ = 0;
  HIP_OK(hipMemcpy(sb.data(), B.batch_bound, (size_t)bc * 8, hipMemcpyDeviceToHost)); HIP_OK(hipMemcpy(sd.data(), B.batch_depth, (size_t)bc * 4, hipMemcpyDeviceToHost));
  HIP_OK(hipMemcpy(&io_, B.inc_obj, 8, hipMemcpyDeviceToHost)); HIP_OK(hipMemcpy(&md_, B.inst_mode, 4, hipMemcpyDeviceToHost));
  std::vector<int> ord(bc); for (int k = 0; k < bc; ++k) ord[k] = k;
  std::sort(ord.begin(), ord.end(), [&](int a, int b) { return sd[a] != sd[b] ? sd[a] > sd[b] : sb[a] < sb[b]; });
  std::fprintf(stderr, "[sel] r%d mode %d incumbent %a:", rounds, md_, io_);
  for (int k : ord) std::fprintf(stderr, " %d.%d/%a", sd[k] >> 6, sd[k] & 63, sb[k]);
  std::fprintf(stderr, "\n");
  return true;
}

inline bool trace_batch(const DevCtx& X, int rounds, int bc) {
  const DevBuf& B = X.B; hipStream_t st = X.stream;
  HIP_OK(hipStreamSynchronize(st));
  if (X.stream2) HIP_OK(hipStreamSynchronize(X.stream2));
  std::vector<int> hd(bc), hi(bc), hk(bc); std::vector<double> ho(bc), hb(bc), hv(bc);
  HIP_OK(hipMemcpy(hd.data(), B.batch_depth, bc * 4, hipMemcpyDeviceToHost)); HIP_OK(hipMemcpy(hi.data(), B.batch_it, bc * 4, hipMemcpyDeviceToHost));
  HIP_OK(hipMemcpy(hk.data(), B.batch_ok, bc * 4, hipMemcpyDeviceToHost)); HIP_OK(hipMemcpy(ho.data(), B.batch_obj, bc * 8, hipMemcpyDeviceToHost));
  HIP_OK(hipMemcpy(hb.data(), B.batch_bound, bc * 8, hipMemcpyDeviceToHost)); HIP_OK(hipMemcpy(hv.data(), B.batch_viol, bc * 8, hipMemcpyDeviceToHost));
  std::vector<int> ord(bc); for (int k = 0; k < bc; ++k) ord[k] = k;
  std::sort(ord.begin(), ord.end(), [&](int a, int b) { return hd[a] != hd[b] ? hd[a] < hd[b] : (ho[a] != ho[b] ? ho[a] < ho[b] : hi[a] < hi[b]); });
  { int oc_ = 0, fc_ = 0, tk_ = 0, dm_ = 0; double nt_ = 0;
    HIP_OK(hipMemcpy(&oc_, B.open_count, 4, hipMemcpyDeviceToHost)); if (B.far_cap > 0) HIP_OK(hipMemcpy(&fc_, B.far_count, 4, hipMemcpyDeviceToHost));
    HIP_OK(hipMemcpy(&nt_, B.near_thr, 8, hipMemcpyDeviceToHost)); HIP_OK(hipMemcpy(&tk_, B.slot_take, 4, hipMemcpyDeviceToHost)); HIP_OK(hipMemcpy(&dm_, B.slot_demand, 4, hipMemcpyDeviceToHost));
    std::fprintf(stderr, "[lists] r%d batch %d: near list after selection %d, far tier %d, near_thr %g, share of the next round %d, demand %d\n", rounds, bc, oc_, fc_, nt_, tk_, dm_); }
  for (int k : ord) std::fprintf(stderr, "[trace] r%d depth %d.%d ok %d it %d obj %a bound %a viol %.3e\n", rounds, hd[k] >> 6, hd[k] & 63, hk[k], hi[k], ho[k], hb[k], hv[k]);
  return true;
}

inline bool trace_launches(const DevCtx& X, int rounds, int bc, size_t nev) {
  const DevBuf& B = X.B; hipStream_t st = X.stream;
  HIP_OK(hipStreamSynchronize(st));
  float m1 = 0, m2 = 0; HIP_OK(hipEventElapsedTime(&m1, X.ipm_ev[nev], X.ev_mid)); HIP_OK(hipEventElapsedTime(&m2, X.ev_mid, X.ipm_ev[nev + 1]));
  int oc = 0; HIP_OK(hipMemcpy(&oc, B.ovf_count, 4, hipMemcpyDeviceToHost));
  std::vector<int> ol(std::max(oc, 1)), hit(bc), hdw(bc), hok(bc);
  if (oc > 0) HIP_OK(hipMemcpy(ol.data(), B.ovf_list, (size_t)oc * 4, hipMemcpyDeviceToHost));
  HIP_OK(hipMemcpy(hit.data(), B.batch_it, (size_t)bc * 4, hipMemcpyDeviceToHost)); HIP_OK(hipMemcpy(hdw.data(), B.batch_depth, (size_t)bc * 4, hipMemcpyDeviceToHost));
  HIP_OK(hipMemcpy(hok.data(), B.batch_ok, (size_t)bc * 4, hipMemcpyDeviceToHost));
  int np = 0, mxp = 0, mxo = 0, mxc = 0; long long sp = 0, so = 0, sc = 0;
  for (int q = 0; q < oc; ++q) { const int k = ol[q]; if ((hdw[k] & 63) == 63 && (hdw[k] >> 6) >= 1) { np++; sp += hit[k]; mxp = std::max(mxp, hit[k]); } else { so += hit[k]; mxo = std::max(mxo, hit[k]); } }
  std::vector<char> isov(bc, 0); for (int q = 0; q < oc; ++q) isov[ol[q]] = 1;
  for (int k = 0; k < bc; ++k) if (!isov[k]) { sc += hit[k]; mxc = std::max(mxc, hit[k]); }
  std::fprintf(stderr, "[launch] round %d nodes %d: on-chip %.2f ms (%d nodes, mean it %.1f, max %d); behind it %.2f ms: %d probes (mean it %.1f, max %d), %d others (mean it %.1f, max %d)\n",
               rounds, bc, m1, bc - oc, (double)sc / std::max(1, bc - oc), mxc, m2, np, (double)sp / std::max(1, np), mxp, oc - np, (double)so / std::max(1, oc - np), mxo);
  return true;
}

inline bool replay_batch(DevCtx& X, int bc) {
  static int replay = process_switches().replay;
  if (replay <= 0) return true;
  const DevBuf& B = X.B; hipStream_t st = X.stream; const Layout& Y = X.Y; (void)Y;
  hipEvent_t e0, e1; HIP_OK(hipEventCreate(&e0)); HIP_OK(hipEventCreate(&e1));
  HIP_OK(hipEventRecord(e0, st));
  for (int r = 0; r < replay; ++r) launch_ipm_batch(X, B, bc, st);
  HIP_OK(hipEventRecord(e1, st)); HIP_OK(hipStreamSynchronize(st));
  float ms = 0; HIP_OK(hipEventElapsedTime(&ms, e0, e1));
  std::vector<int> its(bc); HIP_OK(hipMemcpy(its.data(), B.batch_it, (size_t)bc * 4, hipMemcpyDeviceToHost));
  long long tot = 0; for (int v : its) tot += v;
  std::fprintf(stderr, "[miqp_gpu replay] %d nodes, %lld node-iterations: %.3f ms per pass, %.1f ns per node-iteration\n", bc, tot, ms / replay, 1e6 * ms / replay / (double)tot);
#ifdef MIQP_ABLATE
  if (X.oc_grid > 0 && Y.C == 2) {
    const size_t l_oc = (size_t)oc_lds_layout(Y.N, Y.fixlen).total;
    auto run = [&](auto kern, int mask) {
      HIP_OK(hipFuncSetAttribute((const void*)kern, hipFuncAttributeMaxDynamicSharedMemorySize, (int)l_oc));
      auto once = [&] { (void)hipMemsetAsync(B.work_counter, 0, 4, st); (void)hipMemsetAsync(B.ovf_count, 0, 4, st); hipLaunchKernelGGL(kern, dim3(std::min(bc, X.oc_grid)), dim3(64), l_oc, st, B); };
      once(); HIP_OK(hipEventRecord(e0, st)); for (int r = 0; r < 3; ++r) once(); HIP_OK(hipEventRecord(e1, st)); HIP_OK(hipStreamSynchronize(st));
      float m2 = 0; HIP_OK(hipEventElapsedTime(&m2, e0, e1));
      std::fprintf(stderr, "[miqp_gpu ablate] mask %4d: %.3f ms per pass of %d nodes x 15 iterations = %.1f ns per node-iteration\n", mask, m2 / 3, bc, 1e6 * m2 / 3 / (bc * 15.0));
      return true;
    };
    run(ipm_onchip_kernel<2, OC_NSL, 1>, 1); run(ipm_onchip_kernel<2, OC_NSL, 3>, 3); run(ipm_onchip_kernel<2, OC_NSL, 5>, 5); run(ipm_onchip_kernel<2, OC_NSL, 9>, 9);
    run(ipm_onchip_kernel<2, OC_NSL, 17>, 17); run(ipm_onchip_kernel<2, OC_NSL, 33>, 33); run(ipm_onchip_kernel<2, OC_NSL, 65>, 65); run(ipm_onchip_kernel<2, OC_NSL, 129>, 129);
    run(ipm_onchip_kernel<2, OC_NSL, 257>, 257); run(ipm_onchip_kernel<2, OC_NSL, 513>, 513); run(ipm_onchip_kernel<2, OC_NSL, 1023>, 1023);
    run(ipm_onchip_kernel<2, OC_NSL, 1025>, 1025);
    launch_ipm_batch(X, B, bc, st);
  }
#endif
  replay = 0;
  return true;
}

inline bool print_progress(const DevCtx& X, double t, int rounds, long long launched_nodes, double const0) {
  const DevBuf& B = X.B; hipStream_t st = X.stream;
  double lb0 = 0, io0 = 0; int oc0 = 0; unsigned long long k0 = 0;
  HIP_OK(hipMemcpyAsync(&lb0, B.lower_bound, 8, hipMemcpyDeviceToHost, st)); HIP_OK(hipMemcpyAsync(&io0, B.inc_obj, 8, hipMemcpyDeviceToHost, st));
  HIP_OK(hipMemcpyAsync(&oc0, B.open_count, 4, hipMemcpyDeviceToHost, st)); HIP_OK(hipMemcpyAsync(&k0, B.inc_key, 8, hipMemcpyDeviceToHost, st));
  int fc0 = 0; HIP_OK(hipMemcpyAsync(&fc0, B.far_count, 4, hipMemcpyDeviceToHost, st));
  HIP_OK(hipStreamSynchronize(st));
  std::fprintf(stderr, "[miqp_gpu] t %.2f s round %d nodes %lld: instance 0 bound %.4f incumbent %.4f open %d + %d\n", t, rounds, launched_nodes, lb0, k0 >= 0xFFF0000000000000ull ? INFINITY : io0 + const0, oc0, fc0);
  return true;
}

inline bool dump_open_list(const DevCtx& X, const char* dp, int rounds, int NS, double const0) {
  const DevBuf& B = X.B; const Layout& Y = X.Y; const int open_cap = X.open_cap;
  int oc0 = 0; HIP_OK(hipMemcpy(&oc0, B.open_count, 4, hipMemcpyDeviceToHost)); oc0 = std::min(oc0, open_cap);
  const size_t src = ((size_t)(rounds & 1) * NS + 0) * open_cap;
  std::vector<double> hb(oc0); std::vector<int> hn(oc0), hd(oc0);
  if (oc0 > 0) { HIP_OK(hipMemcpy(hb.data(), B.open_bound + src, (size_t)oc0 * 8, hipMemcpyDeviceToHost)); HIP_OK(hipMemcpy(hn.data(), B.open_node + src, (size_t)oc0 * 4, hipMemcpyDeviceToHost));
    HIP_OK(hipMemcpy(hd.data(), B.open_depth + src, (size_t)oc0 * 4, hipMemcpyDeviceToHost)); }
  std::vector<int> ord(oc0); for (int k = 0; k < oc0; ++k) ord[k] = k;
  std::sort(ord.begin(), ord.end(), [&](int x, int y) { return hb[x] < hb[y]; });
  if (FILE* f = std::fopen(dp, "w")) {
    std::fprintf(f, "%d %d %d %d %d %d %d\n", oc0, Y.fixlen, Y.f_reg, Y.f_env, Y.f_obs, Y.f_c2c, Y.N);
    std::vector<signed char> rec(Y.fixlen);
    for (int q = 0; q < std::min(oc0, 400); ++q) {
      int k = ord[q]; HIP_OK(hipMemcpy(rec.data(), B.pool_fix + (size_t)hn[k] * Y.fixlen, Y.fixlen, hipMemcpyDeviceToHost));
      std::fprintf(f, "%.9g %d", hb[k] + const0, hd[k] >> 6); for (int x = 0; x < Y.fixlen; ++x) std::fprintf(f, " %d", (int)rec[x]); std::fprintf(f, "\n");
    }
    std::fclose(f);
  }
  return true;
}

#ifdef MIQP_PROFILE
inline bool print_profile(const DevCtx& X) {
  const DevBuf& B = X.B;
  { unsigned long long pf[64]; HIP_OK(hipMemcpy(pf, B.prof + 64, 64 * 8, hipMemcpyDeviceToHost));
    const char* nm[10] = {"decode", "rowpass", "bw.phi", "bw.TS+p", "bw.readlane+LDL", "bw.Ksolve", "bw.update", "forward", "step", "update"};
    double tot = 0; for (int q = 0; q < 10; ++q) tot += (double)pf[q];
    { unsigned long long po[16]; HIP_OK(hipMemcpy(po, B.prof, 16 * 8, hipMemcpyDeviceToHost));
      const char* no[9] = {"build", "bw.rows/assemble", "bw.mfma", "bw.TS", "bw.cholK", "bw.P", "forward", "step", "update"};
      double to = 0; for (int q = 0; q < 9; ++q) to += (double)po[q];
      if (po[10]) { std::fprintf(stderr, "[miqp_gpu profile] memory-backed kernel nodes %llu iters %llu cycles/node-iter %.0f :", po[10], po[9], to / std::max(1ull, po[9]));
        for (int q = 0; q < 9; ++q) std::fprintf(stderr, " %s %.1f%% (%.0f)", no[q], 100.0 * po[q] / to, (double)po[q] / std::max(1ull, po[9]));
        std::fprintf(stderr, "; inside bw.TS, the stage-Hessian chain: weights + staging %.0f, single-entry rows %.0f, MFMA loop %.0f, reductions + diagonal %.0f", (double)po[12] / std::max(1ull, po[9]), (double)po[13] / std::max(1ull, po[9]), (double)po[14] / std::max(1ull, po[9]), (double)po[15] / std::max(1ull, po[9]));
        std::fprintf(stderr, "\n"); } }
    std::fprintf(stderr, "[miqp_gpu profile] on-chip nodes %llu iters %llu cycles/node-iter %.0f :", pf[11], pf[10], tot / std::max(1ull, pf[10]));
    for (int q = 0; q < 10; ++q) std::fprintf(stderr, " %s %.1f%% (%.0f)", nm[q], 100.0 * pf[q] / tot, (double)pf[q] / std::max(1ull, pf[10]));
    std::fprintf(stderr, "\n");
    { unsigned long long pa[14]; HIP_OK(hipMemcpy(pa, B.prof + 80, 14 * 8, hipMemcpyDeviceToHost));
      const char* na[9] = {"decode", "gains + first iterate", "scan", "response of the row", "q", "directions + ratio test + M update", "iterate refresh", "results", "warm start"};
      double ta = 0; for (int q = 0; q < 9; ++q) ta += (double)pa[q];
      if (pa[10]) { std::fprintf(stderr, "[miqp_gpu profile] active-set kernel nodes %llu steps %llu cycles/node %.0f :", pa[10], pa[11], ta / (double)pa[10]);
        for (int q = 0; q < 9; ++q) std::fprintf(stderr, " %s %.1f%% (%.0f)", na[q], 100.0 * pa[q] / ta, (double)pa[q] / (double)pa[10]);
        std::fprintf(stderr, "; inside the decode: bound classes %.0f, general-row pass %.0f", (double)pa[12] / (double)pa[10], (double)pa[13] / (double)pa[10]);
        std::fprintf(stderr, "\n");
        unsigned long long pw[3], pl[6]; HIP_OK(hipMemcpy(pw, B.prof + 94, 3 * 8, hipMemcpyDeviceToHost)); HIP_OK(hipMemcpy(pl, B.prof + 120, 6 * 8, hipMemcpyDeviceToHost));
        if (pw[2] && pw[1] && pl[5]) std::fprintf(stderr, "[miqp_gpu profile] standard active-set launches: %llu wavefronts resident %.0f shader cycles = %.1f us each (shader clock %.0f MHz); per launch (%llu folded): span %.3f ms, from the first wavefront out of work to the last end %.3f ms, wavefronts %.0f, resident wavefront time / (span x wavefronts) %.3f\n",
          pw[2], (double)pw[0] / pw[2], (double)pw[1] / pw[2] / 100.0, 100.0 * (double)pw[0] / (double)pw[1], pl[5], (double)pl[3] / pl[5] / 1e5, (double)pl[4] / pl[5] / 1e5, (double)pw[2] / pl[5], ((double)pw[1]) / ((double)pl[3] * ((double)pw[2] / pl[5])));
        unsigned long long ph[16]; HIP_OK(hipMemcpy(ph, B.prof + 128, 16 * 8, hipMemcpyDeviceToHost));
        if (pw[2]) { std::fprintf(stderr, "[miqp_gpu profile] standard active-set wavefronts by their start after the launch's first (< 0.05 / 0.2 / 0.5 / 1 / 2 / 4 / 8 ms / later), %% :");
          for (int q = 0; q < 8; ++q) std::fprintf(stderr, " %.1f", 100.0 * ph[q] / pw[2]);
          std::fprintf(stderr, "; by the nodes they solved (0 / <= 4 / <= 16 / <= 32 / <= 64 / more), %% :");
          for (int q = 8; q < 14; ++q) std::fprintf(stderr, " %.1f", 100.0 * ph[q] / pw[2]);
          std::fprintf(stderr, "\n"); }
        if (const char* wd = X.sw.wave_dump) {
          std::vector<unsigned long long> w(4 * 4 * 4096); HIP_OK(hipMemcpy(w.data(), B.prof + 160, w.size() * 8, hipMemcpyDeviceToHost));
          if (FILE* f = std::fopen(wd, "w")) { for (int q = 0; q < 4 * 4096; ++q) if (w[4 * q]) std::fprintf(f, "%d %llu %llu %u %u %llu %d\n", q & 4095, w[4 * q], w[4 * q + 1], (unsigned)(w[4 * q + 2] >> 32), (unsigned)w[4 * q + 2], w[4 * q + 3], q >> 12); std::fclose(f); } } } }
    { unsigned long long pe[8]; HIP_OK(hipMemcpy(pe, B.prof + 100, 8 * 8, hipMemcpyDeviceToHost));
      const char* ne[6] = {"load", "regions", "leaf disjunctions", "branching", "lifting + reservation", "records"};
      double te = 0; for (int q = 0; q < 6; ++q) te += (double)pe[q];
      if (pe[6]) { std::fprintf(stderr, "[miqp_gpu profile] eval_kernel, %llu branched nodes, cycles/node %.0f :", pe[6], te / (double)pe[6]);
        for (int q = 0; q < 6; ++q) std::fprintf(stderr, " %s %.1f%% (%.0f)", ne[q], 100.0 * pe[q] / te, (double)pe[q] / (double)pe[6]);
        std::fprintf(stderr, "\n"); } }
    { unsigned long long ps[10]; HIP_OK(hipMemcpy(ps, B.prof + 110, 10 * 8, hipMemcpyDeviceToHost));
      const char* ns[8] = {"incumbent copy / kill", "setup", "pass 1 (prune, keys)", "far refill", "bound reduce + spill select", "focus + window + share", "radix select + ties", "pass 3 (emit, compact)"};
      double ts = 0; for (int q = 0; q < 8; ++q) ts += (double)ps[q];
      if (ps[8]) { std::fprintf(stderr, "[miqp_gpu profile] select_kernel, %llu workgroups that reached the end (thread 0's clock), mean list %.0f entries, cycles each %.0f :", ps[8], (double)ps[9] / (double)ps[8], ts / (double)ps[8]);
        for (int q = 0; q < 8; ++q) std::fprintf(stderr, " %s %.1f%% (%.0f)", ns[q], 100.0 * ps[q] / ts, (double)ps[q] / (double)ps[8]);
        std::fprintf(stderr, "\n"); } }
    HIP_OK(hipMemset(B.prof, 0, 160 * 8)); }
  return true;
}
#endif

inline bool print_stats(const DevCtx& X) {
  const DevBuf& B = X.B; const Layout& Y = X.Y;
  unsigned long long hs[256]; HIP_OK(hipMemcpy(hs, B.stats, sizeof(hs), hipMemcpyDeviceToHost)); HIP_OK(hipMemset(B.stats, 0, sizeof(hs)));
  const double nn_ = (double)std::max(1ull, hs[0]);
  std::fprintf(stderr, "[miqp_gpu stats] on-chip nodes %llu (general rows %.1f, coefficients %.1f, box keys %.1f, iterations %.1f per node), handed over %llu; general rows / 32 histogram:", hs[0], hs[1] / nn_, hs[4] / nn_, hs[2] / nn_, hs[5] / nn_, hs[3]);
  for (int q = 0; q < 16; ++q) std::fprintf(stderr, " %llu", hs[8 + q]);
  std::fprintf(stderr, "\n");
  std::fprintf(stderr, "[miqp_gpu stats] node outcomes: infeasible %llu (%.1f it), cut off %llu (%.1f it), not converged %llu (%.1f it), solved %llu (%.1f it) of which: bound >= incumbent %llu, within gap %llu, integer feasible %llu, branched %llu (%.2f children; by kind region/env/obstacle/car-car: %llu x %.1f, %llu x %.1f, %llu x %.1f, %llu x %.1f)\n",
               hs[32], hs[36] / (double)std::max(1ull, hs[32]), hs[33], hs[37] / (double)std::max(1ull, hs[33]), hs[34], hs[38] / (double)std::max(1ull, hs[34]), hs[35], hs[39] / (double)std::max(1ull, hs[35]),
               hs[40], hs[41], hs[42], hs[43], hs[44] / (double)std::max(1ull, hs[43]), hs[48], hs[52] / (double)std::max(1ull, hs[48]), hs[49], hs[53] / (double)std::max(1ull, hs[49]),
               hs[50], hs[54] / (double)std::max(1ull, hs[50]), hs[51], hs[55] / (double)std::max(1ull, hs[51]));
  std::fprintf(stderr, "[miqp_gpu stats] region sets: tightened at %llu (car, step) sites, %llu nodes closed because a step had no region left; children not created because of their lifted bound %llu (multi-row lift larger than the single-row one: %llu), car/car sets tightened at %llu groups\n", hs[58], hs[59], hs[56], hs[57], hs[61]);
  std::fprintf(stderr, "[miqp_gpu stats] region branchings flagged by: own rows %llu (worst class acc box %llu, jerk box %llu, sector %llu, half-plane %llu, curvature %llu, slow square %llu), environment front rows %llu, obstacle front rows %llu, car/car front rows %llu; by step:",
               hs[64], hs[70], hs[71], hs[72], hs[73], hs[74], hs[75], hs[65], hs[66], hs[67]);
  for (int q = 0; q < 32 && q < Y.N; ++q) std::fprintf(stderr, " %llu", hs[160 + q]);
  std::fprintf(stderr, "\n[miqp_gpu stats] node outcomes by origin (processed: infeasible / cut off / not converged / solved):");
  const char* on_[16] = {"root|reg-ref", "reg-adjacent", "reg-other", "reg-slow", "env-ref", "env-other", "-", "-", "obs-ref", "obs-other", "-", "-", "c2c-ref", "c2c-other", "-", "probe"};
  for (int q = 0; q < 16; ++q) if (hs[80 + q]) std::fprintf(stderr, " %s %llu: %llu / %llu / %llu / %llu;", on_[q], hs[80 + q], hs[96 + q], hs[112 + q], hs[128 + q], hs[144 + q]);
  std::fprintf(stderr, "\n[miqp_gpu stats] infeasible rounding probes re-rounded: %llu", hs[62]);
  std::fprintf(stderr, "\n[miqp_gpu stats] handed-over nodes with >= 480 general rows: %llu, mean %.0f, most %llu general rows", hs[7], (double)hs[6] / std::max(1ull, hs[7]), hs[5]);
  std::fprintf(stderr, "\n[miqp_gpu stats] rounding probes by iterations / 3 (0-2, 3-5, ..., 45+):");
  { const char* oc_n[4] = {"infeasible", "cut off", "not converged", "solved"};
    for (int o = 0; o < 4; ++o) { std::fprintf(stderr, " %s", oc_n[o]); for (int q = 0; q < 16; ++q) std::fprintf(stderr, " %llu", hs[192 + 16 * o + q]); std::fprintf(stderr, ";"); } }
  std::fprintf(stderr, "\n");
  return true;
}

inline void print_as_stats(const unsigned long long* h_as) {
  std::fprintf(stderr, "[miqp_gpu stats] active-set launch: %llu nodes (%.1f steps, %.1f drops, %.1f rows from the parent's active set, %.1f active rows at the end per node; %llu infeasible, %llu cut off; %llu started from the parent's M, %llu fell back to a cold start), %llu handed to the interior point (no free slot %llu, step cap %llu, curvature %llu, down-date pivot %llu, rows off their equalities %llu, other %llu); M rebuilt because: the parent left none %llu, the ring had come round %llu, another row count %llu; in the larger block %llu nodes (%.1f steps), of them leaves of the local search %llu (%.1f steps), rounding probes %llu; by their general rows (<= 64 / 96 / 128 / 192 / more) %llu / %llu / %llu / %llu / %llu\n",
               h_as[0], h_as[1] / (double)std::max(1ull, h_as[0]), h_as[3] / (double)std::max(1ull, h_as[0]), h_as[7] / (double)std::max(1ull, h_as[0]), h_as[6] / (double)std::max(1ull, h_as[0]), h_as[4], h_as[5], h_as[8], h_as[9], h_as[2], h_as[11], h_as[12], h_as[13], h_as[14], h_as[15], h_as[10], h_as[17], h_as[18], h_as[19], h_as[20], h_as[21] / (double)std::max(1ull, h_as[20]), h_as[22], h_as[23] / (double)std::max(1ull, h_as[22]), h_as[29], h_as[24], h_as[25], h_as[26], h_as[27], h_as[28]);
}
```

planner_miqp_amd/wrapper.py:

```python
import ctypes as C
import enum
import os
import subprocess

import numpy as np

os.environ.setdefault("GPU_MAX_HW_QUEUES", "8")

from .ctypes_types import (Certificate, CertificateC, FixedResultC, ModelParameters, ModelParamsC, RawResults, RawResultsC, SolutionPropertiesC, SolverOptsC,
                           c_double_p)

_HERE = os.path.dirname(os.path.abspath(__file__))
_LIB = None
EXCHANGE_FN = C.CFUNCTYPE(C.c_int, C.c_void_p, C.c_int, C.c_void_p, C.c_int, C.c_int)


def library_path():
    return os.environ.get("MIQP_GPU_LIB", os.path.join(_HERE, "libmiqp_gpu.so"))


def build_library(force=False):
    src = os.path.join(_HERE, "csrc", "miqp_gpu.hip")
    out = library_path()
    deps = [os.path.join(_HERE, "csrc", f) for f in os.listdir(os.path.join(_HERE, "csrc"))]
    deps += [os.path.join(_HERE, "..", "include", f) for f in ("miqp_gpu.h", "miqp_types.h")]
    if not force and os.path.exists(out) and all(os.path.getmtime(out) >= os.path.getmtime(d) for d in deps):
        return out
    hipcc = os.environ.get("HIPCC", "/opt/rocm/bin/hipcc")
    cmd = [hipcc, "--offload-arch=gfx950", "-O3", "-fno-math-errno", "-fno-trapping-math",
           "-Xarch_device", "-freciprocal-math", "-Xarch_device", "-fno-signed-zeros",
           "-fPIC", "-shared", "-std=c++17", "-o", out, src]
    subprocess.check_call(cmd)
    return out


def load_library():
    global _LIB
    if _LIB is not None:
        return _LIB
    path = library_path()
    if not os.path.exists(path):
        raise RuntimeError("libmiqp_gpu.so is not built (run __graft_entry__.build()); the solver has no CPU fallback")
    L = C.CDLL(path)
    vp = C.c_void_p
    L.miqp_solver_create.restype = vp; L.miqp_solver_create.argtypes = [C.POINTER(SolverOptsC)]
    L.miqp_solver_destroy.restype = None; L.miqp_solver_destroy.argtypes = [vp]
    L.miqp_solver_set_params.restype = C.c_int; L.miqp_solver_set_params.argtypes = [vp, C.POINTER(ModelParamsC)]
    L.miqp_solver_load_dat.restype = C.c_int; L.miqp_solver_load_dat.argtypes = [vp, C.c_char_p]
    L.miqp_solver_override_settings.restype = C.c_int; L.miqp_solver_override_settings.argtypes = [vp, C.c_double, C.c_double]
    L.miqp_solver_set_warmstart.restype = C.c_int; L.miqp_solver_set_warmstart.argtypes = [vp, C.POINTER(RawResultsC), C.c_int]
    L.miqp_solver_solve.restype = C.c_int; L.miqp_solver_solve.argtypes = [vp, C.c_double]
    L.miqp_solver_solve_batch.restype = C.c_int; L.miqp_solver_solve_batch.argtypes = [C.POINTER(vp), C.c_int, C.POINTER(C.c_int)]
    L.miqp_solver_solve_stream.restype = C.c_int; L.miqp_solver_solve_stream.argtypes = [C.POINTER(vp), C.c_int, C.c_int, C.POINTER(C.c_int)]
    L.miqp_solver_solve_batch_multi.restype = C.c_int; L.miqp_solver_solve_batch_multi.argtypes = [C.POINTER(vp), C.c_int, C.c_int, C.POINTER(C.c_int)]
    L.miqp_solver_raw_sizes.restype = C.c_int; L.miqp_solver_raw_sizes.argtypes = [vp, C.POINTER(C.c_int)]
    L.miqp_solver_lift_tables.restype = C.c_int; L.miqp_solver_lift_tables.argtypes = [vp, c_double_p, C.c_int]
    L.miqp_solver_solve_split.restype = C.c_int; L.miqp_solver_solve_split.argtypes = [vp, C.c_double, C.c_int, C.c_int, EXCHANGE_FN, vp]
    L.miqp_solver_solve_split_rccl.restype = C.c_int; L.miqp_solver_solve_split_rccl.argtypes = [vp, C.c_double]
    L.miqp_solver_split_roots.restype = C.c_int
    L.miqp_solver_split_roots.argtypes = [vp, C.c_int, C.c_int, C.POINTER(C.c_int), C.POINTER(C.c_int), C.POINTER(C.c_int), C.c_int, C.POINTER(C.c_int), C.POINTER(C.c_int)]
    L.miqp_comm_unique_id.restype = C.c_int; L.miqp_comm_unique_id.argtypes = [C.c_char_p]
    L.miqp_comm_init.restype = C.c_int; L.miqp_comm_init.argtypes = [C.c_int, C.c_int, C.c_char_p, C.c_int]
    L.miqp_comm_finalize.restype = C.c_int; L.miqp_comm_finalize.argtypes = []
    L.miqp_comm_selftest.restype = C.c_int; L.miqp_comm_selftest.argtypes = [EXCHANGE_FN, vp, C.c_int, C.c_int]
    L.miqp_solver_get_results.restype = C.c_int; L.miqp_solver_get_results.argtypes = [vp, C.POINTER(RawResultsC)]
    L.miqp_solver_materialize_results.restype = C.c_int; L.miqp_solver_materialize_results.argtypes = [C.POINTER(vp), C.c_int, C.c_int]
    L.miqp_solver_get_properties.restype = C.c_int; L.miqp_solver_get_properties.argtypes = [vp, C.POINTER(SolutionPropertiesC)]
    L.miqp_solver_get_dims.restype = C.c_int; L.miqp_solver_get_dims.argtypes = [vp, C.POINTER(C.c_int)]
    L.miqp_solver_export_lp.restype = C.c_int; L.miqp_solver_export_lp.argtypes = [vp, C.c_char_p]
    for fn in (L.miqp_solver_write_dat, L.miqp_solver_write_solution, L.miqp_solver_write_mst, L.miqp_solver_read_mst):
        fn.restype = C.c_int; fn.argtypes = [vp, C.c_char_p]
    L.miqp_solver_solve_fixed.restype = C.c_int
    L.miqp_solver_solve_fixed.argtypes = [vp, C.POINTER(RawResultsC), C.POINTER(RawResultsC), C.POINTER(C.c_double), C.POINTER(C.c_int)]
    L.miqp_solver_last_timing.restype = C.c_int; L.miqp_solver_last_timing.argtypes = [vp, C.POINTER(C.c_double)]
    L.miqp_solver_last_setup.restype = C.c_int; L.miqp_solver_last_setup.argtypes = [vp, C.POINTER(C.c_double)]
    L.miqp_solver_last_active_set.restype = C.c_int; L.miqp_solver_last_active_set.argtypes = [vp, C.POINTER(C.c_double)]
    L.miqp_solver_last_fixed_route.restype = C.c_int; L.miqp_solver_last_fixed_route.argtypes = [vp]
    L.miqp_solver_last_error.restype = C.c_char_p; L.miqp_solver_last_error.argtypes = [vp]
    L.miqp_solver_last_admission.restype = C.c_int; L.miqp_solver_last_admission.argtypes = [vp, C.POINTER(C.c_double)]
    L.miqp_solver_certify.restype = C.c_int; L.miqp_solver_certify.argtypes = [vp, C.POINTER(RawResultsC), C.POINTER(CertificateC)]
    L.miqp_solver_certify_batch.restype = C.c_int; L.miqp_solver_certify_batch.argtypes = [C.POINTER(vp), C.c_int, C.POINTER(CertificateC)]
    L.miqp_gpu_certificate_size.restype = C.c_int; L.miqp_gpu_certificate_size.argtypes = []
    L.miqp_gpu_certify_last_timing.restype = C.c_int; L.miqp_gpu_certify_last_timing.argtypes = [C.POINTER(C.c_double)]
    L.miqp_gpu_has_active_set.restype = C.c_int; L.miqp_gpu_has_active_set.argtypes = [C.c_int, C.c_int]
    L.miqp_solver_launch_plan.restype = C.c_int
    L.miqp_solver_launch_plan.argtypes = [vp, C.c_int, C.c_int, C.c_int, C.POINTER(C.c_int), C.c_int, C.c_double, C.c_int, C.POINTER(C.c_int), C.c_int]
    L.miqp_solver_solve_fixed_batch.restype = C.c_int
    L.miqp_solver_solve_fixed_batch.argtypes = [vp, C.POINTER(C.POINTER(RawResultsC)), C.c_int, C.POINTER(FixedResultC), C.POINTER(C.c_int)]
    L.miqp_solver_fixed_batch_record.restype = C.c_int; L.miqp_solver_fixed_batch_record.argtypes = [vp, C.c_int, C.POINTER(RawResultsC)]
    L.miqp_gpu_fixed_result_size.restype = C.c_int; L.miqp_gpu_fixed_result_size.argtypes = []
    L.miqp_gpu_fixed_batch_chunk.restype = C.c_int; L.miqp_gpu_fixed_batch_chunk.argtypes = []
    L.miqp_solver_set_pool.restype = C.c_int; L.miqp_solver_set_pool.argtypes = [vp, C.c_int]
    L.miqp_solver_pool_count.restype = C.c_int; L.miqp_solver_pool_count.argtypes = [vp]
    L.miqp_solver_pool_found.restype = C.c_int; L.miqp_solver_pool_found.argtypes = [vp, c_double_p, C.c_int]
    L.miqp_solver_pool_solve.restype = C.c_int; L.miqp_solver_pool_solve.argtypes = [vp, C.POINTER(FixedResultC), C.c_int]
    L.miqp_solver_pool_record.restype = C.c_int; L.miqp_solver_pool_record.argtypes = [vp, C.c_int, C.POINTER(RawResultsC)]
    L.miqp_gpu_pool_max.restype = C.c_int; L.miqp_gpu_pool_max.argtypes = []
    L.miqp_solver_set_pool_filter.restype = C.c_int; L.miqp_solver_set_pool_filter.argtypes = [vp, C.c_int]
    L.miqp_gpu_pool_signature.restype = C.c_int
    L.miqp_gpu_pool_signature.argtypes = [C.c_int, C.c_int, C.c_int, C.c_int, C.POINTER(C.c_byte), C.POINTER(C.c_byte), C.c_int]
    L.miqp_solver_pool_signature.restype = C.c_int; L.miqp_solver_pool_signature.argtypes = [vp, C.POINTER(RawResultsC), C.c_int, C.POINTER(C.c_byte), C.c_int]
    L.miqp_solver_pool_found_decisions.restype = C.c_int; L.miqp_solver_pool_found_decisions.argtypes = [vp, C.c_int, C.POINTER(C.c_byte), C.c_int]
    L.miqp_solver_solve_fixed_multi.restype = C.c_int
    L.miqp_solver_solve_fixed_multi.argtypes = [C.POINTER(vp), C.c_int, C.POINTER(C.POINTER(RawResultsC)), C.POINTER(C.c_int), C.POINTER(FixedResultC), C.POINTER(C.c_int)]
    L.miqp_solver_pool_solve_multi.restype = C.c_int
    L.miqp_solver_pool_solve_multi.argtypes = [C.POINTER(vp), C.c_int, C.POINTER(FixedResultC), C.c_int, C.POINTER(C.c_int)]
    if L.miqp_gpu_fixed_result_size() != C.sizeof(FixedResultC):
        raise RuntimeError("libmiqp_gpu.so and ctypes_types.FixedResultC disagree on miqp_fixed_result_c (%d / %d bytes): rebuild the library"
                           % (L.miqp_gpu_fixed_result_size(), C.sizeof(FixedResultC)))
    L.miqp_gpu_version.restype = C.c_char_p
    _LIB = L
    return L


EXPORTED_SYMBOLS = ["miqp_solver_create", "miqp_solver_destroy", "miqp_solver_set_params", "miqp_solver_load_dat",
                    "miqp_solver_override_settings", "miqp_solver_set_warmstart", "miqp_solver_solve",
                    "miqp_solver_solve_batch", "miqp_solver_get_results", "miqp_solver_get_properties",
                    "miqp_solver_get_dims", "miqp_solver_export_lp", "miqp_solver_solve_fixed",
                    "miqp_solver_last_timing", "miqp_solver_last_active_set", "miqp_solver_last_setup", "miqp_solver_last_error", "miqp_solver_last_admission", "miqp_gpu_version", "miqp_solver_write_dat", "miqp_solver_write_solution",
                    "miqp_solver_write_mst", "miqp_solver_read_mst", "miqp_fraction_parameters", "miqp_mean_angles",
                    "miqp_limits_per_region", "miqp_calculate_region_idx", "miqp_reserve_neighbor_regions",
                    "miqp_calculate_possible_regions", "miqp_calculate_warmstart", "miqp_plan",
                    "miqp_solver_solve_batch_multi", "miqp_solver_raw_sizes", "miqp_solver_lift_tables", "miqp_reference_trajectory", "miqp_update_car", "miqp_fitting_polynomial_parameters",
                    "miqp_solver_solve_split", "miqp_solver_solve_split_rccl", "miqp_solver_split_roots", "miqp_comm_unique_id",
                    "miqp_comm_init", "miqp_comm_finalize", "miqp_comm_selftest", "miqp_solver_solve_stream", "miqp_solver_materialize_results",
                    "miqp_initial_pose_check", "miqp_select_environment", "miqp_obstacle_intersects_environment", "miqp_obstacles_roi", "miqp_bark_trajectory", "miqp_obstacle_intersects_environment_roi", "miqp_environment_warmstart",
                    "miqp_solver_certify", "miqp_solver_certify_batch", "miqp_gpu_certificate_size", "miqp_gpu_certify_last_timing",
                    "miqp_gpu_has_active_set", "miqp_solver_last_fixed_route", "miqp_solver_launch_plan",
                    "miqp_solver_solve_fixed_batch", "miqp_solver_fixed_batch_record", "miqp_gpu_fixed_result_size", "miqp_gpu_fixed_batch_chunk",
                    "miqp_solver_set_pool", "miqp_solver_pool_count", "miqp_solver_pool_found", "miqp_solver_pool_solve", "miqp_solver_pool_record", "miqp_gpu_pool_max",
                    "miqp_solver_solve_fixed_multi", "miqp_solver_pool_solve_multi",
                    "miqp_solver_set_pool_filter", "miqp_gpu_pool_signature", "miqp_solver_pool_signature", "miqp_solver_pool_found_decisions"]


LAUNCH_PLAN_FIELDS = ("kernel", "stream", "grid", "lds", "ovf_mode", "cls_take", "as_split", "skip_probes", "bounce", "work", "from_ovf2", "bufs", "zero")


_FIXED_RESULT_DTYPE = np.dtype([("status", "<i4"), ("route", "<i4"), ("iterations", "<i4"), ("reserved", "<i4"), ("objective", "<f8"), ("violation", "<f8")])


POOL_BY_REGION, POOL_BY_ENVIRONMENT, POOL_BY_OBSTACLE, POOL_BY_CAR_CAR, POOL_EXACT_TIMING = 1, 2, 4, 8, 16


def _decision_len(cars, steps, obstacles):
    return cars * steps * 6 + cars * obstacles * steps * 5 + cars * (cars - 1) // 2 * steps * 4


def pool_signature(cars, steps, obstacles, families, decisions):
    d = np.ascontiguousarray(decisions, dtype=np.int8)
    D = _decision_len(int(cars), int(steps), int(obstacles))
    if d.ndim != 1 or d.size < D or D <= 0:
        raise ValueError("%d decision bytes given, the shape has %d" % (d.size, D))
    out = np.empty(D, dtype=np.int8)
    bp = C.POINTER(C.c_byte)
    rc = load_library().miqp_gpu_pool_signature(int(cars), int(steps), int(obstacles), int(families), d.ctypes.data_as(bp), out.ctypes.data_as(bp), D)
    if rc != D:
        raise ValueError("miqp_gpu_pool_signature refused the arguments (%d)" % rc)
    return out


def pool_max():
    return int(load_library().miqp_gpu_pool_max())


def fixed_batch_chunk():
    return int(load_library().miqp_gpu_fixed_batch_chunk())


def has_active_set(cars, steps):
    return int(load_library().miqp_gpu_has_active_set(int(cars), int(steps)))


class OptimizationStatus(enum.IntEnum):
    SUCCESS = 0
    FAILED_NO_SOLUT = 1
    FAILED_SEG_FAULT = 2
    FAILED_TIMEOUT = 3


class WarmstartType(enum.IntEnum):
    NO_WARMSTART = 0
    RECEDING_HORIZON_WARMSTART = 1
    LAST_SOLUTION_WARMSTART = 2
    BOTH_WARMSTART_STRATEGIES = 3


class ParameterSource(enum.IntEnum):
    DATFILE = 0
    CPPINPUTS = 1
    MIXED = 2


class SolutionProperties:
    def __init__(self, c=None):
        for n, _ in SolutionPropertiesC._fields_:
            setattr(self, n, getattr(c, n) if c is not None else 0)

    def __repr__(self):
        return "SolutionProperties(" + ", ".join("%s=%r" % (n, getattr(self, n)) for n, _ in SolutionPropertiesC._fields_) + ")"


class CplexWrapper:

    def __init__(self, modfile="cplexmodel.mod", parameterSource=ParameterSource.CPPINPUTS, precision=12, modpath="cplexmodel/",
                 nodes_per_round=0, max_open_nodes=0, gap_override=-1.0, verbose=0, device=-1):
        self._L = load_library()
        self._opts = SolverOptsC(int(precision), int(device), int(nodes_per_round), int(max_open_nodes), float(gap_override), int(verbose))
        self._h = self._L.miqp_solver_create(C.byref(self._opts))
        self.parameterSource_ = ParameterSource(parameterSource)
        self.modfile_ = modpath + modfile
        self.datfile_ = ""
        self._params = None
        self._keep = None
        self._results = None
        self._warm = None
        self.useSpecialOrderedSets_ = False
        self.useBranchingPriorities_ = False
        self.doWarmstart_ = WarmstartType.NO_WARMSTART
        self.debugOutputFilePath_ = ""
        self.debugOutputFilePrefix_ = ""
        self.print_debug_outputs_ = False
        self.debugOutputParameterFilePath_ = ""
        self.tmpWarmstartFile_ = "/tmp/warmstart_debug_res.mst"

    def __del__(self):
        try:
            if self._h:
                self._L.miqp_solver_destroy(self._h)
                self._h = None
        except Exception:
            pass

    def setParameterDatFileRelative(self, datfile):
        self.datfile_ = "cplexmodel/" + datfile

    def setParameterDatFileAbsolute(self, datfile):
        self.datfile_ = datfile

    def resetParameters(self, parameters: ModelParameters):
        self._params = parameters

    def overrideSolverSettingsDataSource(self, parameters: ModelParameters):
        if self._params is not None:
            for n in ["max_solution_time", "relative_mip_gap_tolerance", "mipdisplay", "mipemphasis", "relobjdif", "cutpass",
                      "probe", "repairtries", "rinsheur", "varsel", "mircuts", "parallelmode"]:
                setattr(self._params, n, getattr(parameters, n))

    def setSpecialOrderedSets(self, v):
        self.useSpecialOrderedSets_ = bool(v)

    def setUseBranchingPriorities(self, v):
        self.useBranchingPriorities_ = bool(v)

    def setBranchingPriorityValueExtent(self, value, extent):
        self.branchingPriority_ = (value, extent)

    def setBufferCplexOutputsToStream(self, v):
        pass

    def setDebugOutputPrint(self, v):
        self.print_debug_outputs_ = bool(v)

    def setDebugOutputFilePath(self, p):
        self.debugOutputFilePath_ = p

    def setDebugOutputFilePrefix(self, p):
        self.debugOutputFilePrefix_ = p

    def addRecedingHorizonWarmstart(self, warmstart: RawResults, wt=WarmstartType.RECEDING_HORIZON_WARMSTART):
        self.doWarmstart_ = wt if wt == WarmstartType.RECEDING_HORIZON_WARMSTART else WarmstartType.BOTH_WARMSTART_STRATEGIES
        self._warm = warmstart

    def setLastSolutionWarmstart(self, wt=WarmstartType.LAST_SOLUTION_WARMSTART):
        self.doWarmstart_ = wt if wt == WarmstartType.LAST_SOLUTION_WARMSTART else WarmstartType.BOTH_WARMSTART_STRATEGIES

    def deleteLastSolutionWarmstartFile(self):
        self._last = None
        if os.path.exists(self.tmpWarmstartFile_):
            os.remove(self.tmpWarmstartFile_)

    def _push_inputs(self):
        if self.parameterSource_ == ParameterSource.DATFILE:
            rc = self._L.miqp_solver_load_dat(self._h, self.datfile_.encode())
        elif self.parameterSource_ == ParameterSource.MIXED and self._params is None:
            rc = self._L.miqp_solver_load_dat(self._h, self.datfile_.encode())
        else:
            if self._params is None:
                return -1
            s, self._keep = self._params.to_c()
            rc = self._L.miqp_solver_set_params(self._h, C.byref(s))
        if rc != 0:
            return rc
        self._L.miqp_solver_set_warmstart(self._h, None, int(WarmstartType.NO_WARMSTART))
        if self.doWarmstart_ in (WarmstartType.RECEDING_HORIZON_WARMSTART, WarmstartType.BOTH_WARMSTART_STRATEGIES) and self._warm is not None:
            wc = self._warm.to_c()
            self._L.miqp_solver_set_warmstart(self._h, C.byref(wc), int(WarmstartType.RECEDING_HORIZON_WARMSTART))
        if self.doWarmstart_ in (WarmstartType.LAST_SOLUTION_WARMSTART, WarmstartType.BOTH_WARMSTART_STRATEGIES):
            if os.path.exists(self.tmpWarmstartFile_):
                self._L.miqp_solver_read_mst(self._h, self.tmpWarmstartFile_.encode())
        return 0

    def _stamp(self, timestamp):
        return "%.15g" % float(timestamp)

    def _debug_before(self, timestamp):
        if not self.print_debug_outputs_:
            return
        base = os.path.join(self.debugOutputFilePath_, self.debugOutputFilePrefix_)
        self.debugOutputParameterFilePath_ = base + "parameters_" + self._stamp(timestamp) + ".txt"
        self._L.miqp_solver_write_dat(self._h, self.debugOutputParameterFilePath_.encode())
        self._L.miqp_solver_export_lp(self._h, (base + "lpexport_" + self._stamp(timestamp) + ".lp").encode())

    def _debug_after(self, timestamp, status):
        if status != OptimizationStatus.SUCCESS:
            return
        last = self.doWarmstart_ in (WarmstartType.LAST_SOLUTION_WARMSTART, WarmstartType.BOTH_WARMSTART_STRATEGIES)
        if last:
            self._L.miqp_solver_write_mst(self._h, self.tmpWarmstartFile_.encode())
        if self.print_debug_outputs_:
            base = os.path.join(self.debugOutputFilePath_, self.debugOutputFilePrefix_)
            self._L.miqp_solver_write_solution(self._h, (base + "solution_" + self._stamp(timestamp) + ".txt").encode())
            if last:
                self._L.miqp_solver_write_mst(self._h, (base + "warmstartsolution_" + self._stamp(timestamp) + ".mst").encode())

    def _collect(self, status, lazy=False):
        self._stale = status == OptimizationStatus.SUCCESS
        if not self._stale:
            return OptimizationStatus(status)
        if not lazy:
            self._fetch()
        return OptimizationStatus(status)

    def _fetch(self):
        if getattr(self, "_stale", False):
            d = (C.c_int * 6)()
            self._L.miqp_solver_get_dims(self._h, d)
            res = RawResults(*list(d))
            rc = res.to_c()
            if self._L.miqp_solver_get_results(self._h, C.byref(rc)) != 0:
                raise RuntimeError("miqp_solver_get_results failed: the library holds no solution for this handle")
            self._results = res
            self._last = res
            self._stale = False

    def callCplex(self, timestamp=0.0):
        if self._push_inputs() != 0:
            return OptimizationStatus.FAILED_SEG_FAULT
        self._debug_before(timestamp)
        st = self._collect(self._L.miqp_solver_solve(self._h, float(timestamp)))
        self._debug_after(timestamp, st)
        return st

    def callCplexSplit(self, world, rank, exchange=None, timestamp=0.0):
        if self._push_inputs() != 0:
            return OptimizationStatus.FAILED_SEG_FAULT
        if exchange is None:
            st = self._L.miqp_solver_solve_split_rccl(self._h, float(timestamp))
        else:
            st = self._L.miqp_solver_solve_split(self._h, float(timestamp), int(world), int(rank), exchange, None)
        return self._collect(st)

    def splitRoots(self, world, rank):
        if self._push_inputs() != 0:
            return None
        cap = 4096
        ro, ix, va = (C.c_int * cap)(), (C.c_int * cap)(), (C.c_int * cap)()
        nr, nc = C.c_int(0), C.c_int(0)
        n = self._L.miqp_solver_split_roots(self._h, int(world), int(rank), ro, ix, va, cap, C.byref(nr), C.byref(nc))
        if n < 0:
            return None
        roots = [[] for _ in range(nr.value)]
        for k in range(min(n, cap)):
            roots[ro[k]].append((ix[k], va[k]))
        return roots, nc.value

    def getRawResults(self):
        self._fetch()
        return self._results

    def getSolutionProperties(self):
        p = SolutionPropertiesC()
        self._L.miqp_solver_get_properties(self._h, C.byref(p))
        return SolutionProperties(p)

    def getTmpWarmstartFile(self):
        return self.tmpWarmstartFile_

    def getDebugOutputParameterFilePath(self):
        return self.debugOutputParameterFilePath_

    def writeDat(self, path):
        if self._push_inputs() != 0:
            return -1
        return self._L.miqp_solver_write_dat(self._h, path.encode())

    def solveFixed(self, fixed: RawResults):
        if self._push_inputs() != 0:
            return None
        d = (C.c_int * 6)()
        self._L.miqp_solver_get_dims(self._h, d)
        out = RawResults(*list(d))
        oc = out.to_c()
        fc = fixed.to_c()
        obj = C.c_double(0)
        it = C.c_int(0)
        rc = self._L.miqp_solver_solve_fixed(self._h, C.byref(fc), C.byref(oc), C.byref(obj), C.byref(it))
        return rc, out, obj.value, it.value

    def lastFixedRoute(self):
        return int(self._L.miqp_solver_last_fixed_route(self._h))

    def launchPlan(self, bc, overlap=0, par=-1, cls_n=(-1, -1, -1), cus=256, free_gb=256.0, as_on=1, concurrent=True):
        if self._push_inputs() != 0:
            return None
        out = (C.c_int * (5 * len(LAUNCH_PLAN_FIELDS)))()
        n = self._L.miqp_solver_launch_plan(self._h, int(bc), int(overlap), int(par), (C.c_int * 3)(*cls_n), int(cus), float(free_gb),
                                            (1 if as_on else 0) | (0 if concurrent else 2), out, len(out))
        if n < 0:
            raise RuntimeError("miqp_solver_launch_plan failed (%d)" % n)
        k = len(LAUNCH_PLAN_FIELDS)
        return [tuple(out[i * k:(i + 1) * k]) for i in range(n)]

    def solveFixedBatch(self, records):
        if self._push_inputs() != 0:
            raise RuntimeError("invalid parameters")
        n = len(records)
        keep = [r.to_c() if r is not None else None for r in records]
        ptrs = (C.POINTER(RawResultsC) * max(n, 1))(*[C.pointer(c) if c is not None else None for c in keep])
        out = (FixedResultC * max(n, 1))()
        best = C.c_int(-1)
        rc = self._L.miqp_solver_solve_fixed_batch(self._h, ptrs, n, out, C.byref(best))
        if rc != 0:
            raise RuntimeError("miqp_solver_solve_fixed_batch failed (%d)" % rc)
        a = np.frombuffer(out, dtype=np.dtype([("status", "<i4"), ("route", "<i4"), ("iterations", "<i4"), ("reserved", "<i4"),
                                               ("objective", "<f8"), ("violation", "<f8")]), count=n)
        return (a["status"].copy(), a["objective"].copy(), a["violation"].copy(), a["iterations"].copy(), a["route"].copy(), best.value)

    def fixedBatchRecord(self, k):
        d = (C.c_int * 6)()
        if self._L.miqp_solver_get_dims(self._h, d) != 0:
            return -1, None
        out = RawResults(*list(d))
        oc = out.to_c()
        rc = self._L.miqp_solver_fixed_batch_record(self._h, int(k), C.byref(oc))
        return rc, (out if rc == 0 else None)

    def setSolutionPool(self, capacity):
        return int(self._L.miqp_solver_set_pool(self._h, int(capacity)))

    def setSolutionPoolFilter(self, families):
        return int(self._L.miqp_solver_set_pool_filter(self._h, int(families)))

    def solutionPoolFoundDecisions(self, k):
        d = (C.c_int * 6)()
        if self._L.miqp_solver_get_dims(self._h, d) != 0:
            return None
        out = np.empty(_decision_len(d[0], d[1], d[4]), dtype=np.int8)
        rc = self._L.miqp_solver_pool_found_decisions(self._h, int(k), out.ctypes.data_as(C.POINTER(C.c_byte)), out.size)
        return out if rc == out.size else None

    def poolSignature(self, record, families):
        d = (C.c_int * 6)()
        if self._L.miqp_solver_get_dims(self._h, d) != 0 and (self._push_inputs() != 0 or self._L.miqp_solver_get_dims(self._h, d) != 0):
            raise ValueError("invalid parameters")
        out = np.empty(_decision_len(d[0], d[1], d[4]), dtype=np.int8)
        rc = self._L.miqp_solver_pool_signature(self._h, C.byref(record.to_c()), int(families), out.ctypes.data_as(C.POINTER(C.c_byte)), out.size)
        if rc != out.size:
            raise ValueError("miqp_solver_pool_signature refused the arguments (%d)" % rc)
        return out

    def solutionPoolCount(self):
        return int(self._L.miqp_solver_pool_count(self._h))

    def solutionPoolFound(self):
        n = self.solutionPoolCount()
        o = np.zeros(max(n, 1))
        m = self._L.miqp_solver_pool_found(self._h, o.ctypes.data_as(c_double_p), n)
        return o[:max(m, 0)].copy()

    def solveSolutionPool(self):
        n = max(self.solutionPoolCount(), 1)
        out = (FixedResultC * n)()
        m = self._L.miqp_solver_pool_solve(self._h, out, n)
        if m < 0:
            raise RuntimeError("miqp_solver_pool_solve failed (%d)" % m)
        a = np.frombuffer(out, dtype=np.dtype([("status", "<i4"), ("route", "<i4"), ("iterations", "<i4"), ("reserved", "<i4"),
                                               ("objective", "<f8"), ("violation", "<f8")]), count=m)
        return (a["status"].copy(), a["objective"].copy(), a["violation"].copy(), a["iterations"].copy(), a["route"].copy())

    def solutionPoolRecord(self, k):
        d = (C.c_int * 6)()
        if self._L.miqp_solver_get_dims(self._h, d) != 0:
            return -1, None
        out = RawResults(*list(d))
        oc = out.to_c()
        rc = self._L.miqp_solver_pool_record(self._h, int(k), C.byref(oc))
        return rc, (out if rc == 0 else None)

    def liftTables(self):
        if self._push_inputs() != 0:
            raise RuntimeError("invalid parameters")
        p = self._params
        out = np.zeros((p.NumCars, 2, p.NumSteps, 4, 4))
        n = self._L.miqp_solver_lift_tables(self._h, out.ctypes.data_as(c_double_p), out.size)
        if n != out.size:
            raise RuntimeError("miqp_solver_lift_tables failed (%d)" % n)
        return out

    def rawSizes(self):
        if self._push_inputs() != 0:
            return None
        o = (C.c_int * 4)()
        if self._L.miqp_solver_raw_sizes(self._h, o) != 0:
            return None
        return dict(rows=o[0], bin=o[1], cont=o[2], nnz=o[3])

    def certify(self, candidate: RawResults = None, use_real_slack=True):
        out = CertificateC()
        if candidate is None:
            rc = self._L.miqp_solver_certify(self._h, None, C.byref(out))
        else:
            d = (C.c_int * 6)()
            if self._L.miqp_solver_get_dims(self._h, d) != 0 and self._push_inputs() != 0:
                raise RuntimeError("invalid parameters")
            cc = candidate.to_c()
            if not use_real_slack:
                cc.slackvars_real = None
            rc = self._L.miqp_solver_certify(self._h, C.byref(cc), C.byref(out))
        if rc != 0:
            raise RuntimeError("miqp_solver_certify failed (%d): %s" % (rc, self.lastError()))
        return Certificate(out)

    def lastAdmission(self):
        o = (C.c_double * 1)()
        self._L.miqp_solver_last_admission(self._h, o)
        return o[0]

    def lastError(self):
        return (self._L.miqp_solver_last_error(self._h) or b"").decode()

    def lastTiming(self):
        t = (C.c_double * 6)()
        self._L.miqp_solver_last_timing(self._h, t)
        u = (C.c_double * 3)()
        self._L.miqp_solver_last_setup(self._h, u)
        v = (C.c_double * 8)()
        self._L.miqp_solver_last_active_set(self._h, v)
        return dict(solve_s=t[0], ipm_s=t[1], ipm_launches=int(t[2]), nodes=int(t[3]), ipm_iters=int(t[4]), row_iters=int(t[5]),
                    setup_s=u[0], context_s=u[1], context_built=bool(u[2]),
                    as_nodes=int(v[0]), as_steps=int(v[1]), as_unfinished=int(v[2]), as_drops=int(v[3]), as_rows_end=int(v[4]), as_rows_parent=int(v[5]),
                    std_launch_s=v[6], std_launches=int(v[7]))


def prepare_batch(wrappers):
    for w in wrappers:
        if w._push_inputs() != 0:
            raise RuntimeError("invalid parameters")


def solve_batch(wrappers, gpus=None, inflight=None, prepared=False):
    L = load_library()
    if not prepared:
        prepare_batch(wrappers)
    n = len(wrappers)
    hs = (C.c_void_p * n)(*[w._h for w in wrappers])
    st = (C.c_int * n)(*([int(OptimizationStatus.FAILED_SEG_FAULT)] * n))
    if inflight is not None and gpus is None:
        rc = L.miqp_solver_solve_stream(hs, n, int(inflight), st)
    else:
        rc = L.miqp_solver_solve_batch(hs, n, st) if gpus is None else L.miqp_solver_solve_batch_multi(hs, n, int(gpus), st)
    if rc not in (0, -2):
        return [OptimizationStatus.FAILED_SEG_FAULT] * n
    return [w._collect(st[k], lazy=True) for k, w in enumerate(wrappers)]

# ... 70 lines not shown
```

Before: 1079.

## Walk fixed-decision sites in active-set decode instead of testing every slot

The active-set kernel's decode policy now enables a site-walk mode by default. It enumerates only the constraint slots the fixed decisions can activate (per-car region, environment and obstacle sites, plus pair sites), rather than testing every slot with slot_maybe. A reciprocal-multiply division (oc_rcp) appears to replace integer division when recovering the stage from a code, and a host-side exhaustive check of that trick is added. The change also adds a decode probe kernel, host APIs and Python wrappers for comparing walk and non-walk outputs, plus finer profiling counters. The risk is a mismatch between the walked site set and the full test, which would yield different candidate rows.

```diff
diff --git a/include/miqp_gpu.h b/include/miqp_gpu.h
--- a/include/miqp_gpu.h
+++ b/include/miqp_gpu.h
@@ -104,6 +104,14 @@
 
 int miqp_solver_launch_plan(const miqp_solver_t* s, int bc, int overlap, int par, const int* cls_n3, int cus, double free_gb, int flags, int* out, int cap);
 
+int miqp_solver_decode_probe(miqp_solver_t* s, const miqp_raw_results_c* const* fixed, int n, const signed char* c2n, int big, int walk, unsigned char* out, int cap);
+
+int miqp_solver_fix_record(const miqp_solver_t* s, const miqp_raw_results_c* rec, signed char* out, int cap, int* shape6);
+
+int miqp_gpu_decode_sites(int cars, int steps, int pieces, int piece_edges, int obstacles, int obstacle_edges, const signed char* fix, int fixlen, int which, unsigned short* out, int cap);
+
+int miqp_gpu_decode_rcp_check(void);
+
 int miqp_solver_last_setup(const miqp_solver_t* s, double* out3);
 
 int miqp_solver_last_admission(const miqp_solver_t* s, double* out1);
diff --git a/planner_miqp_amd/csrc/as_onchip.hip b/planner_miqp_amd/csrc/as_onchip.hip
--- a/planner_miqp_amd/csrc/as_onchip.hip
+++ b/planner_miqp_amd/csrc/as_onchip.hip
@@ -17,10 +17,15 @@
 
 template <int C> __device__ inline int as_col(int pq) { return C == 2 ? ((pq & 3) << 2) | (pq >> 2) : ((pq & 1) << 2) | (pq >> 1); }
 template <int C> __device__ inline int as_pcol(int q) { return C == 2 ? ((q & 3) << 2) | (q >> 2) : ((q & 3) << 1) | (q >> 2); }
-template <int C> struct AsDecode {
-  static constexpr bool LANE_BOUNDS = true, ROW_IDENTITY = true, MARKS = true;
+template <int C, bool WALK, bool MARKS_ = false> struct AsDecodeT {
+  static constexpr bool LANE_BOUNDS = true, ROW_IDENTITY = true, MARKS = MARKS_, SITE_WALK = WALK;
   static __device__ int col(int l) { return as_col<C>(oc_pcol<C, true>(l)); }
 };
+#ifdef OC_DECODE_OLD_WALK
+template <int C> using AsDecode = AsDecodeT<C, false, true>;
+#else
+template <int C> using AsDecode = AsDecodeT<C, true, true>;
+#endif
 
 template <int C, int NSL, int GCAP = miqp::OC_GCAP>
 __global__ void __launch_bounds__(64, (GCAP > 128 ? 1 : 2)) as_onchip_kernel(DevBuf B) {
@@ -110,7 +115,7 @@
     }
 
 #ifdef MIQP_PROFILE
-    unsigned long long asp_[12] = {0, 0, 0, 0, 0, 0, 0, 0, 0, 0, 0, 0};
+    unsigned long long asp_[13] = {0, 0, 0, 0, 0, 0, 0, 0, 0, 0, 0, 0, 0};
 #endif
     ASP_T(ta0);
 #define OC_DECODE_POLICY AsDecode<C>
@@ -130,6 +135,7 @@
     ASP_T(ta1); ASP_ACC(0, ta0, ta1);
 #ifdef MIQP_PROFILE
     asp_[9] += (unsigned long long)(ocd_t_sparse - ta0); asp_[11] += (unsigned long long)(ta1 - ocd_t_rows);
+    asp_[10] += (unsigned long long)ocd_t_flush; asp_[12] += (unsigned long long)(ocd_t_rows - ocd_t_walked);
 #endif
     double brhs[NSL];
     unsigned int bact = 0u, binA = 0u, ginA = 0u;
@@ -597,7 +603,7 @@
       ++wv_nodes;
       { const long long tc1 = clock64(); asp_[7] += (unsigned long long)(tc1 - tc0);
         for (int q_ = 0; q_ < 9; ++q_) atomicAdd(&B.prof[80 + q_], asp_[q_]);
-        atomicAdd(&B.prof[92], asp_[9]); atomicAdd(&B.prof[93], asp_[11]);
+        atomicAdd(&B.prof[92], asp_[9]); atomicAdd(&B.prof[93], asp_[11]); atomicAdd(&B.prof[97], asp_[10]); atomicAdd(&B.prof[98], asp_[12]);
         atomicAdd(&B.prof[90], 1ull); atomicAdd(&B.prof[91], (unsigned long long)steps); }
 #endif
       if (B.as_stats) {
diff --git a/planner_miqp_amd/csrc/decode_probe.hip b/planner_miqp_amd/csrc/decode_probe.hip
--- /dev/null
+++ b/planner_miqp_amd/csrc/decode_probe.hip
@@ -0,0 +1,195 @@
+#pragma once
+
+namespace miqp {
+
+struct DecodeProbeOut { int head, sstart, bkey, cand, gmeta, gcoef, grhs, total; };
+__host__ __device__ inline DecodeProbeOut decode_probe_layout(int N, int gcap) {
+  DecodeProbeOut P; int o = 0;
+  P.head = o; o += 16;
+  P.sstart = o; o += ((N + 2) * 4 + 7) & ~7;
+  P.bkey = o; o += N * 32 * 8;
+  P.cand = o; o += (gcap * 2 + 7) & ~7;
+  P.gmeta = o; o += gcap * 16;
+  P.gcoef = o; o += oc_gcoef_of(gcap) * 8;
+  P.grhs = o; o += gcap * 8;
+  P.total = o;
+  return P;
+}
+
+struct DecodeProbeArgs { Layout Y; const double* D; const int* T; const signed char* fix; unsigned char* out; int n; };
+
+template <int C, bool WALK, int GCAP>
+__global__ void __launch_bounds__(64) decode_probe_kernel(const DecodeProbeArgs A) {
+  constexpr int OC_GCAP = GCAP, OC_GCOEF = oc_gcoef_of(GCAP), NZ = 8 * C;
+  const Layout& Y = A.Y;
+  const double* D = A.D; const int* T = A.T;
+  const int tid = threadIdx.x, N = Y.N, NSLOT = Y.NSLOT;
+  const unsigned long long lt = (1ull << tid) - 1ull;
+  if ((int)blockIdx.x >= A.n) return;
+  extern __shared__ double lds[];
+  char* const L0 = (char*)lds;
+  const OcLds LL = oc_lds_layout(N, Y.fixlen, OC_GCAP, GCAP == miqp::OC_GCAP);
+  double* const scr = (double*)(L0 + LL.u);
+  unsigned long long* const bkey = (unsigned long long*)(L0 + LL.r);
+  uint4* const gmeta = (uint4*)(L0 + LL.gmeta);
+  double* const gcoef = (double*)(L0 + LL.gcoef);
+  double* const grhs = (double*)(L0 + LL.grhs);
+  int* const sstart = (int*)(L0 + LL.sstart);
+  unsigned short* const cand = (unsigned short*)(L0 + LL.cand);
+  signed char* const fix = (signed char*)(L0 + LL.fix);
+  {
+    const signed char* src = A.fix + (size_t)blockIdx.x * Y.fixlen;
+    for (int k = tid; k < Y.fixlen; k += 64) fix[k] = src[k];
+    for (int k = tid; k < N * 32; k += 64) bkey[k] = ~0ull;
+    for (int k = tid; k <= N + 1; k += 64) sstart[k] = 0;
+  }
+  __syncthreads();
+#define OC_DECODE_POLICY AsDecodeT<C, WALK>
+#include "oc_decode_body.inc"
+#undef OC_DECODE_POLICY
+  OC_WAVE_SYNC();
+  const DecodeProbeOut P = decode_probe_layout(N, GCAP);
+  unsigned char* const o = A.out + (size_t)blockIdx.x * P.total;
+  const int NM = overflow ? 0 : sstart[N + 1];
+  if (tid == 0) { int* h = (int*)(o + P.head); h[0] = ngen; h[1] = overflow ? 1 : 0; h[2] = overflow ? 0 : ncoef; h[3] = NM; }
+  for (int k = tid; k < N * 32; k += 64) ((unsigned long long*)(o + P.bkey))[k] = bkey[k];
+  if (!overflow) {
+    for (int k = tid; k <= N + 1; k += 64) ((int*)(o + P.sstart))[k] = sstart[k];
+    for (int k = tid; k < NM && k < GCAP; k += 64) {
+      ((unsigned short*)(o + P.cand))[k] = cand[k]; ((uint4*)(o + P.gmeta))[k] = gmeta[k]; ((double*)(o + P.grhs))[k] = grhs[k];
+    }
+    for (int k = tid; k < ncoef && k < OC_GCOEF; k += 64) ((double*)(o + P.gcoef))[k] = gcoef[k];
+  }
+}
+
+}
+
+namespace {
+
+template <int C> int decode_sites_host(const Layout& Y, const signed char* fix, int which, unsigned short* out, int cap) {
+  int n = 0;
+  auto put = [&](int code) { if (n < cap) out[n] = (unsigned short)code; ++n; };
+  for (int i = 0; i < Y.N; ++i) {
+    if (which == 0) {
+      for (int slot = 0; slot < Y.NSLOT; ++slot) {
+        if (slot < C * Y.SC && slot % Y.SC < 11) continue;
+        if (miqp::slot_maybe<C>(Y, fix, i, slot)) put(i * Y.NSLOT + slot);
+      }
+    } else {
+      for (int c = 0; c < C; ++c) miqp::car_sites<C>(Y, fix, c, i, put);
+      for (int p = 0; p < Y.NP; ++p) miqp::pair_sites<C>(Y, fix, p, i, put);
+    }
+  }
+  return n;
+}
+
+template <int C, int GCAP> bool decode_probe_launch(bool walk, const miqp::DecodeProbeArgs& A, size_t lds) {
+  auto k0 = miqp::decode_probe_kernel<C, false, GCAP>; auto k1 = miqp::decode_probe_kernel<C, true, GCAP>;
+  HIP_OK(hipFuncSetAttribute((const void*)(walk ? k1 : k0), hipFuncAttributeMaxDynamicSharedMemorySize, (int)lds));
+  if (walk) hipLaunchKernelGGL(k1, dim3(A.n), dim3(64), lds, 0, A); else hipLaunchKernelGGL(k0, dim3(A.n), dim3(64), lds, 0, A);
+  HIP_OK(hipGetLastError());
+  return true;
+}
+
+struct DecodeProbeBufs {
+  double* D = nullptr; int* T = nullptr; signed char* fix = nullptr; unsigned char* out = nullptr;
+  ~DecodeProbeBufs() { if (D) (void)hipFree(D); if (T) (void)hipFree(T); if (fix) (void)hipFree(fix); if (out) (void)hipFree(out); }
+};
+
+bool decode_probe_run(const Layout& Y, const std::vector<double>& D, const std::vector<int>& T, const std::vector<signed char>& fix, int n, bool big, bool walk, unsigned char* out, size_t stride) {
+  DecodeProbeBufs G;
+  HIP_OK(hipMalloc((void**)&G.D, D.size() * 8)); HIP_OK(hipMalloc((void**)&G.T, T.size() * 4));
+  HIP_OK(hipMalloc((void**)&G.fix, fix.size())); HIP_OK(hipMalloc((void**)&G.out, (size_t)n * stride));
+  HIP_OK(hipMemcpy(G.D, D.data(), D.size() * 8, hipMemcpyHostToDevice)); HIP_OK(hipMemcpy(G.T, T.data(), T.size() * 4, hipMemcpyHostToDevice));
+  HIP_OK(hipMemcpy(G.fix, fix.data(), fix.size(), hipMemcpyHostToDevice)); HIP_OK(hipMemset(G.out, 0, (size_t)n * stride));
+  miqp::DecodeProbeArgs A; A.Y = Y; A.D = G.D; A.T = G.T; A.fix = G.fix; A.out = G.out; A.n = n;
+  const size_t lds = (size_t)miqp::oc_lds_layout(Y.N, Y.fixlen, big ? miqp::OC_GCAP_BIG : miqp::OC_GCAP, !big).total;
+  bool ok;
+  if (Y.C == 1) ok = big ? decode_probe_launch<1, miqp::OC_GCAP_BIG>(walk, A, lds) : decode_probe_launch<1, miqp::OC_GCAP>(walk, A, lds);
+  else ok = big ? decode_probe_launch<2, miqp::OC_GCAP_BIG>(walk, A, lds) : decode_probe_launch<2, miqp::OC_GCAP>(walk, A, lds);
+  if (!ok) return false;
+  HIP_OK(hipDeviceSynchronize());
+  HIP_OK(hipMemcpy(out, G.out, (size_t)n * stride, hipMemcpyDeviceToHost));
+  return true;
+}
+
+}
+
+extern "C" {
+
+int miqp_gpu_decode_sites(int cars, int steps, int pieces, int piece_edges, int obstacles, int obstacle_edges, const signed char* fix, int fixlen, int which, unsigned short* out, int cap) {
+  if (cars < 1 || cars > MAXC || steps < 1 || pieces < 0 || piece_edges < 0 || obstacles < 0 || obstacle_edges < 0 || !fix || (!out && cap > 0) || cap < 0 || which < 0 || which > 1) return -1;
+  const Layout Y = make_layout(cars, steps, 1, 1, pieces, piece_edges, obstacles, obstacle_edges);
+  if ((long long)Y.N * Y.NSLOT > 65535) return -2;
+  if (fixlen < Y.fixlen) return -3;
+  switch (cars) {
+    case 1: return decode_sites_host<1>(Y, fix, which, out, cap);
+    case 2: return decode_sites_host<2>(Y, fix, which, out, cap);
+    case 3: return decode_sites_host<3>(Y, fix, which, out, cap);
+    default: return decode_sites_host<4>(Y, fix, which, out, cap);
+  }
+}
+
+int miqp_solver_fix_record(const miqp_solver_t* s, const miqp_raw_results_c* rec, signed char* out, int cap, int* shape6) {
+  if (!s || !s->has_inst || !rec || !fixed_record_ok(*rec) || !dims_match(*rec, s->inst)) return -1;
+  miqp_solver_t* one[1] = {const_cast<miqp_solver_t*>(s)};
+  const BatchShape bs = batch_layout(one, 1);
+  if (!bs.ok) return -2;
+  const Layout& Y = bs.Y;
+  if (shape6) { shape6[0] = Y.C; shape6[1] = Y.N; shape6[2] = Y.E; shape6[3] = Y.EL; shape6[4] = Y.O; shape6[5] = Y.L; }
+  if (!out) return Y.fixlen;
+  if (cap < Y.fixlen) return -4;
+  std::vector<double> D(Y.dstride); std::vector<int> T(Y.istride);
+  compile_instance(s->inst, Y, D.data(), T.data());
+  std::vector<signed char> fix;
+  if (!fix_from_results(s->inst, Y, T.data(), rec, fix)) return -1;
+  std::memcpy(out, fix.data(), (size_t)Y.fixlen);
+  return Y.fixlen;
+}
+
+int miqp_gpu_decode_rcp_check(void) {
+  const int nth = std::max(1, std::min(8, (int)std::thread::hardware_concurrency()));
+  std::atomic<int> next{2}, first_bad{0};
+  auto work = [&] {
+    for (int d0 = next.fetch_add(256); d0 <= 65535; d0 = next.fetch_add(256))
+      for (int d = d0; d < d0 + 256 && d <= 65535; ++d) {
+        const unsigned int r = miqp::oc_rcp(d), ud = (unsigned int)d;
+        unsigned int bad = 0;
+        for (unsigned int code = 0; code < 65536u; ++code) { const unsigned int q = (unsigned int)(((unsigned long long)code * r) >> 32), lo = q * ud; bad |= (unsigned int)(lo > code) | (unsigned int)(code - lo >= ud); }
+        if (bad) { int cur = first_bad.load(); while ((cur == 0 || d < cur) && !first_bad.compare_exchange_weak(cur, d)) {} }
+      }
+  };
+  if (nth <= 1) work();
+  else { std::vector<std::thread> th; for (int t = 0; t < nth; ++t) th.emplace_back(work); for (auto& t : th) t.join(); }
+  return first_bad.load();
+}
+
+int miqp_solver_decode_probe(miqp_solver_t* s, const miqp_raw_results_c* const* fixed, int n, const signed char* c2n, int big, int walk, unsigned char* out, int cap) {
+  if (!s || !s->has_inst || n < 0 || (n > 0 && !fixed)) return -1;
+  miqp_solver_t* one[1] = {s};
+  const BatchShape bs = batch_layout(one, 1);
+  if (!bs.ok || !miqp::as_shape_ok(bs.Y.C, bs.Y.N)) return -2;
+  const Layout& Y = bs.Y;
+  const size_t stride = (size_t)miqp::decode_probe_layout(Y.N, big ? miqp::OC_GCAP_BIG : miqp::OC_GCAP).total;
+  const size_t lds = (size_t)miqp::oc_lds_layout(Y.N, Y.fixlen, big ? miqp::OC_GCAP_BIG : miqp::OC_GCAP, !big).total;
+  if (lds > 160 * 1024 || n > 65536) return -2;
+  if (!out || n == 0) return (int)stride;
+  if ((size_t)cap < (size_t)n * stride) return -4;
+  for (int k = 0; k < n; ++k) if (!fixed[k] || !fixed_record_ok(*fixed[k]) || !dims_match(*fixed[k], s->inst)) return -1;
+  std::vector<double> D(Y.dstride); std::vector<int> T(Y.istride);
+  compile_instance(s->inst, Y, D.data(), T.data());
+  const size_t fl = (size_t)Y.fixlen, nc2n = (size_t)Y.NP * Y.N * 4;
+  std::vector<signed char> fix((size_t)n * fl), one_fix;
+  for (int k = 0; k < n; ++k) {
+    (void)fix_from_results(s->inst, Y, T.data(), fixed[k], one_fix);
+    if (c2n) std::memcpy(one_fix.data() + Y.f_c2n, c2n + (size_t)k * nc2n, nc2n);
+    std::memcpy(fix.data() + (size_t)k * fl, one_fix.data(), fl);
+  }
+  DevCtx* X = ctx_for_device(s->opts.device);
+  if (!X) return -3;
+  std::lock_guard<std::mutex> lk(X->mu);
+  if (hipSetDevice(X->device) != hipSuccess) return -3;
+  return decode_probe_run(Y, D, T, fix, n, big != 0, walk != 0, out, stride) ? (int)stride : -3;
+}
+
+}
diff --git a/planner_miqp_amd/csrc/ipm_onchip.hip b/planner_miqp_amd/csrc/ipm_onchip.hip
--- a/planner_miqp_amd/csrc/ipm_onchip.hip
+++ b/planner_miqp_amd/csrc/ipm_onchip.hip
@@ -29,7 +29,7 @@
 template <int C, bool CM> __device__ inline int oc_pcol(int l) { return (CM && l < 6 * C) ? 2 * C * (l % 3) + l / 3 : l; }
 template <int C, bool CM> __device__ inline int oc_lcol(int p) { return (CM && p < 6 * C) ? 3 * (p % (2 * C)) + p / (2 * C) : p; }
 template <int C, bool CM> struct IpmDecode {
-  static constexpr bool LANE_BOUNDS = false, ROW_IDENTITY = false, MARKS = false;
+  static constexpr bool LANE_BOUNDS = false, ROW_IDENTITY = false, MARKS = false, SITE_WALK = false;
   static __device__ int col(int l) { return oc_pcol<C, CM>(l); }
 };
 template <int CTRL> __device__ inline double dpp_shift0(double x) {
diff --git a/planner_miqp_amd/csrc/miqp_gpu.hip b/planner_miqp_amd/csrc/miqp_gpu.hip
--- a/planner_miqp_amd/csrc/miqp_gpu.hip
+++ b/planner_miqp_amd/csrc/miqp_gpu.hip
@@ -1448,6 +1448,7 @@
 #include "fixed_batch.hip"
 #include "solution_pool.hip"
 #include "fixed_multi.hip"
+#include "decode_probe.hip"
 
 extern "C" {
 
diff --git a/planner_miqp_amd/csrc/oc_decode.hip b/planner_miqp_amd/csrc/oc_decode.hip
--- a/planner_miqp_amd/csrc/oc_decode.hip
+++ b/planner_miqp_amd/csrc/oc_decode.hip
@@ -88,7 +88,7 @@
 }
 
 template <int C>
-__device__ inline bool slot_maybe(const Layout& Y, const signed char* fix, int i, int slot) {
+__host__ __device__ inline bool slot_maybe(const Layout& Y, const signed char* fix, int i, int slot) {
   const int N = Y.N;
   if (slot < C * Y.SC) {
     const int c = slot / Y.SC, rr = slot - c * Y.SC;
@@ -116,4 +116,58 @@
   return m > 0 && ((m >> alt) & 1);
 }
 
+template <int C, class Put>
+__host__ __device__ inline void car_sites(const Layout& Y, const signed char* fix, int c, int i, Put&& put) {
+  if (i < 1) return;
+  const int N = Y.N, base = i * Y.NSLOT + c * Y.SC;
+  const int code = (int)fix[Y.f_reg + c * N + i];
+  const int nreg = code >= 0 ? ((code & 3) != 3 ? 5 : 4) : 2;
+#pragma unroll 1
+  for (int k = 0; k < nreg; ++k) put(base + 11 + k);
+  if (Y.E >= 1) {
+    const signed char* fe = fix + Y.f_env + (c * N + i) * 5;
+#pragma unroll 1
+    for (int pt = 0; pt < 5; ++pt) {
+      const int e = Y.E == 1 ? 0 : (int)fe[pt];
+      if (e >= 0 && (pt == 0 || code >= 0)) {
+#pragma unroll 1
+        for (int k = 0; k < Y.EL; ++k) put(base + 16 + pt * Y.EL + k);
+      }
+    }
+  }
+#pragma unroll 1
+  for (int o = 0; o < Y.O; ++o) {
+    const signed char* fo = fix + Y.f_obs + ((c * Y.O + o) * N + i) * 5;
+#pragma unroll 1
+    for (int pt = 0; pt < 5; ++pt) { const int kk = (int)fo[pt]; if (kk >= 0 && kk < Y.L && (pt == 0 || code >= 0)) put(base + 16 + 5 * Y.EL + o * 5 + pt); }
+  }
 }
+template <int C, class Put>
+__host__ __device__ inline void pair_sites(const Layout& Y, const signed char* fix, int p, int i, Put&& put) {
+  if (C < 2 || i < 1) return;
+  const int N = Y.N, base = i * Y.NSLOT + C * Y.SC;
+  const signed char* fc = fix + Y.f_c2c + (p * N + i) * 4;
+#pragma unroll 1
+  for (int grp = 0; grp < 4; ++grp) if ((int)fc[grp] >= 0) { put(base + p * 8 + grp * 2); put(base + p * 8 + grp * 2 + 1); }
+  const signed char* fn = fix + Y.f_c2n + (p * N + i) * 4;
+#pragma unroll 1
+  for (int grp = 0; grp < 4; ++grp) {
+    const int m = (int)fn[grp];
+    if (m > 0) {
+#pragma unroll 1
+      for (int alt = 0; alt < 4; ++alt) if ((m >> alt) & 1) put(base + Y.NP * 8 + p * 16 + grp * 4 + alt);
+    }
+  }
+}
+__host__ __device__ inline int oc_sites_per_lane_max(const Layout& Y) { const int a = 5 + 5 * Y.EL + 5 * Y.O; return a > 24 ? a : 24; }
+
+__host__ __device__ inline unsigned int oc_rcp(int nslot) { return 0xFFFFFFFFu / (unsigned int)nslot + 1u; }
+__host__ __device__ inline int oc_div_rcp(int code, unsigned int rcp) {
+#if defined(__HIP_DEVICE_COMPILE__)
+  return (int)__umulhi((unsigned int)code, rcp);
+#else
+  return (int)(((unsigned long long)(unsigned int)code * rcp) >> 32);
+#endif
+}
+
+}
diff --git a/planner_miqp_amd/csrc/oc_decode_body.inc b/planner_miqp_amd/csrc/oc_decode_body.inc
--- a/planner_miqp_amd/csrc/oc_decode_body.inc
+++ b/planner_miqp_amd/csrc/oc_decode_body.inc
@@ -1,6 +1,8 @@
 #ifdef MIQP_PROFILE
-    long long ocd_t_sparse = 0, ocd_t_rows = 0;
+    long long ocd_t_sparse = 0, ocd_t_rows = 0, ocd_t_walked = 0, ocd_t_flush = 0;
 #endif
+    const unsigned int ocd_rcp = OC_DECODE_POLICY::SITE_WALK ? oc_rcp(NSLOT) : 0u;
+    auto ocd_stage = [&](int pcode) -> int { if constexpr (OC_DECODE_POLICY::SITE_WALK) return oc_div_rcp(pcode, ocd_rcp); else return pcode / NSLOT; };
     int ngen = 0;
     {
       unsigned long long* const bmp = (unsigned long long*)scr;
@@ -21,10 +23,16 @@
       const int LCAP = (int)(((char*)(L0 + LL.r) - (char*)plist) / 2) - 64;
       int nlist = 0;
       auto flush = [&]() {
+#ifdef MIQP_PROFILE
+        const long long ocd_f0 = OC_DECODE_POLICY::MARKS ? clock64() : 0;
+#endif
         OC_WAVE_SYNC();
-        for (int j0 = 0; j0 < nlist; j0 += 64) if (j0 + tid < nlist) { const int pc = plist[j0 + tid]; const int i = pc / NSLOT; take(i, pc - i * NSLOT); }
+        for (int j0 = 0; j0 < nlist; j0 += 64) if (j0 + tid < nlist) { const int pc = plist[j0 + tid]; const int i = ocd_stage(pc); take(i, pc - i * NSLOT); }
         OC_WAVE_SYNC();
         nlist = 0;
+#ifdef MIQP_PROFILE
+        if (OC_DECODE_POLICY::MARKS) ocd_t_flush += clock64() - ocd_f0;
+#endif
       };
       if constexpr (OC_DECODE_POLICY::LANE_BOUNDS) {
         for (int e0 = 0; e0 < C * N; e0 += 64) {
@@ -60,6 +68,38 @@
           }
         }
       }
+      if constexpr (OC_DECODE_POLICY::SITE_WALK) {
+        static_assert(OC_DECODE_POLICY::LANE_BOUNDS, "the site walk covers the sparse classes only: the bound classes need the lane pass");
+#ifdef MIQP_PROFILE
+        if (OC_DECODE_POLICY::MARKS) ocd_t_sparse = clock64();
+#endif
+        const int PCAP = LCAP + 64 > 64 ? LCAP + 64 : 64;
+        const int nent = (C + Y.NP) * N;
+        for (int e0 = 0; e0 < nent; e0 += 64) {
+          const int e = e0 + tid;
+          const bool in = e < nent;
+          const int ent = in ? e / N : 0, i = e - ent * N;
+          int cnt = 0, end = 0, total = 0, w0 = 0, w1 = 0, base = 0, lo = 0, hi = 0;
+#pragma unroll 1
+          for (int ph = 0;; ++ph) {
+            int pos = base;
+            if (in) {
+              auto put = [&](int code) { if (pos >= lo && pos < hi) plist[pos] = (unsigned short)code; ++pos; };
+              if (ent < C) car_sites<C>(Y, fix, ent, i, put); else pair_sites<C>(Y, fix, ent - C, i, put);
+            }
+            if (ph == 0) {
+              cnt = pos; end = cnt;
+#pragma unroll
+              for (int d = 1; d < 64; d <<= 1) { const int up = __shfl_up(end, d); if (tid >= d) end += up; }
+              total = __builtin_amdgcn_readlane(end, 63);
+            } else { nlist += w1 - w0; w0 = w1; }
+            if (w0 >= total) break;
+            if (nlist >= PCAP) flush();
+            w1 = total - w0 < PCAP - nlist ? total : w0 + PCAP - nlist;
+            base = nlist - w0 + end - cnt; lo = nlist; hi = nlist + w1 - w0;
+          }
+        }
+      } else {
 #pragma unroll 1
       for (int cl = 0; cl < 8; ++cl) {
 #ifdef MIQP_PROFILE
@@ -83,7 +123,11 @@
           if (nlist > LCAP) flush();
         }
       }
+      }
       flush();
+#ifdef MIQP_PROFILE
+      if (OC_DECODE_POLICY::MARKS) ocd_t_walked = clock64();
+#endif
       if (tid == 0) { int a = 0; for (int k = 0; k < nw; ++k) { pre[k] = (unsigned short)(a < 65535 ? a : 65535); a += __popcll(bmp[k]); } pre[nw] = (unsigned short)(a < 65535 ? a : 65535); }
       OC_WAVE_SYNC();
       ngen = pre[nw];
@@ -105,7 +149,7 @@
       int i = 0, nn = 0;
       const bool mine = tid < OC_SCR && c0 + tid < ngen;
       int slot_ = 0;
-      if (mine) { const int pcode = cand[c0 + tid]; i = pcode / NSLOT; slot_ = pcode - i * NSLOT; r = decode_row<C, true>(Y, D, T, fix, i, slot_, g); }
+      if (mine) { const int pcode = cand[c0 + tid]; i = ocd_stage(pcode); slot_ = pcode - i * NSLOT; r = decode_row<C, true>(Y, D, T, fix, i, slot_, g); }
       unsigned long long map = 0ull; unsigned int cols = 0u;
       double v6[6];
 #pragma unroll
diff --git a/planner_miqp_amd/csrc/solve_diag.hpp b/planner_miqp_amd/csrc/solve_diag.hpp
--- a/planner_miqp_amd/csrc/solve_diag.hpp
+++ b/planner_miqp_amd/csrc/solve_diag.hpp
@@ -143,6 +143,9 @@
       if (pa[10]) { std::fprintf(stderr, "[miqp_gpu profile] active-set kernel nodes %llu steps %llu cycles/node %.0f :", pa[10], pa[11], ta / (double)pa[10]);
         for (int q = 0; q < 9; ++q) std::fprintf(stderr, " %s %.1f%% (%.0f)", na[q], 100.0 * pa[q] / ta, (double)pa[q] / (double)pa[10]);
         std::fprintf(stderr, "; inside the decode: bound classes %.0f, general-row pass %.0f", (double)pa[12] / (double)pa[10], (double)pa[13] / (double)pa[10]);
+        { unsigned long long pd[2]; HIP_OK(hipMemcpy(pd, B.prof + 97, 2 * 8, hipMemcpyDeviceToHost));
+          const double sp = (double)pa[0] - (double)pa[12] - (double)pa[13];
+          std::fprintf(stderr, ", sparse classes %.0f = site walk %.0f + full test (flushes) %.0f + candidate list %.0f", sp / (double)pa[10], (sp - (double)pd[0] - (double)pd[1]) / (double)pa[10], (double)pd[0] / (double)pa[10], (double)pd[1] / (double)pa[10]); }
         std::fprintf(stderr, "\n");
         unsigned long long pw[3], pl[6]; HIP_OK(hipMemcpy(pw, B.prof + 94, 3 * 8, hipMemcpyDeviceToHost)); HIP_OK(hipMemcpy(pl, B.prof + 120, 6 * 8, hipMemcpyDeviceToHost));
         if (pw[2] && pw[1] && pl[5]) std::fprintf(stderr, "[miqp_gpu profile] standard active-set launches: %llu wavefronts resident %.0f shader cycles = %.1f us each (shader clock %.0f MHz); per launch (%llu folded): span %.3f ms, from the first wavefront out of work to the last end %.3f ms, wavefronts %.0f, resident wavefront time / (span x wavefronts) %.3f\n",
diff --git a/planner_miqp_amd/wrapper.py b/planner_miqp_amd/wrapper.py
--- a/planner_miqp_amd/wrapper.py
+++ b/planner_miqp_amd/wrapper.py
@@ -85,6 +85,12 @@
     L.miqp_gpu_has_active_set.restype = C.c_int; L.miqp_gpu_has_active_set.argtypes = [C.c_int, C.c_int]
     L.miqp_solver_launch_plan.restype = C.c_int
     L.miqp_solver_launch_plan.argtypes = [vp, C.c_int, C.c_int, C.c_int, C.POINTER(C.c_int), C.c_int, C.c_double, C.c_int, C.POINTER(C.c_int), C.c_int]
+    L.miqp_solver_decode_probe.restype = C.c_int
+    L.miqp_solver_decode_probe.argtypes = [vp, C.POINTER(C.POINTER(RawResultsC)), C.c_int, C.POINTER(C.c_byte), C.c_int, C.c_int, C.POINTER(C.c_ubyte), C.c_int]
+    L.miqp_solver_fix_record.restype = C.c_int; L.miqp_solver_fix_record.argtypes = [vp, C.POINTER(RawResultsC), C.POINTER(C.c_byte), C.c_int, C.POINTER(C.c_int)]
+    L.miqp_gpu_decode_sites.restype = C.c_int
+    L.miqp_gpu_decode_sites.argtypes = [C.c_int] * 6 + [C.POINTER(C.c_byte), C.c_int, C.c_int, C.POINTER(C.c_ushort), C.c_int]
+    L.miqp_gpu_decode_rcp_check.restype = C.c_int; L.miqp_gpu_decode_rcp_check.argtypes = []
     L.miqp_solver_solve_fixed_batch.restype = C.c_int
     L.miqp_solver_solve_fixed_batch.argtypes = [vp, C.POINTER(C.POINTER(RawResultsC)), C.c_int, C.POINTER(FixedResultC), C.POINTER(C.c_int)]
     L.miqp_solver_fixed_batch_record.restype = C.c_int; L.miqp_solver_fixed_batch_record.argtypes = [vp, C.c_int, C.POINTER(RawResultsC)]
@@ -130,7 +136,8 @@
                     "miqp_solver_solve_fixed_batch", "miqp_solver_fixed_batch_record", "miqp_gpu_fixed_result_size", "miqp_gpu_fixed_batch_chunk",
                     "miqp_solver_set_pool", "miqp_solver_pool_count", "miqp_solver_pool_found", "miqp_solver_pool_solve", "miqp_solver_pool_record", "miqp_gpu_pool_max",
                     "miqp_solver_solve_fixed_multi", "miqp_solver_pool_solve_multi",
-                    "miqp_solver_set_pool_filter", "miqp_gpu_pool_signature", "miqp_solver_pool_signature", "miqp_solver_pool_found_decisions"]
+                    "miqp_solver_set_pool_filter", "miqp_gpu_pool_signature", "miqp_solver_pool_signature", "miqp_solver_pool_found_decisions",
+                    "miqp_solver_decode_probe", "miqp_solver_fix_record", "miqp_gpu_decode_sites", "miqp_gpu_decode_rcp_check"]
 
 
 LAUNCH_PLAN_FIELDS = ("kernel", "stream", "grid", "lds", "ovf_mode", "cls_take", "as_split", "skip_probes", "bounce", "work", "from_ovf2", "bufs", "zero")
@@ -157,6 +164,33 @@
     if rc != D:
         raise ValueError("miqp_gpu_pool_signature refused the arguments (%d)" % rc)
     return out
+
+
+def decode_sites(cars, steps, pieces, piece_edges, obstacles, obstacle_edges, fix, generated):
+    f = np.ascontiguousarray(fix, dtype=np.int8)
+    args = [int(cars), int(steps), int(pieces), int(piece_edges), int(obstacles), int(obstacle_edges), f.ctypes.data_as(C.POINTER(C.c_byte)), int(f.size), 1 if generated else 0]
+    L = load_library()
+    n = L.miqp_gpu_decode_sites(*(args + [None, 0]))
+    if n < 0:
+        raise ValueError("miqp_gpu_decode_sites refused the arguments (%d)" % n)
+    out = np.empty(max(n, 1), dtype=np.uint16)
+    if L.miqp_gpu_decode_sites(*(args + [out.ctypes.data_as(C.POINTER(C.c_ushort)), n])) != n:
+        raise RuntimeError("miqp_gpu_decode_sites changed its mind")
+    return np.sort(out[:n])
+
+
+def decode_fix_layout(cars, steps, obstacles):
+    NP = cars * (cars - 1) // 2
+    f_env = cars * steps
+    f_obs = f_env + cars * steps * 5
+    f_c2c = f_obs + cars * obstacles * steps * 5
+    f_c2n = f_c2c + NP * steps * 4
+    f_rmask = f_c2n + NP * steps * 4
+    return 0, f_env, f_obs, f_c2c, f_c2n, f_rmask, (f_rmask + cars * steps * 2 + 15) & ~15
+
+
+def decode_rcp_check():
+    return int(load_library().miqp_gpu_decode_rcp_check())
 
 
 def pool_max():
@@ -420,6 +454,56 @@
             raise RuntimeError("miqp_solver_launch_plan failed (%d)" % n)
         k = len(LAUNCH_PLAN_FIELDS)
         return [tuple(out[i * k:(i + 1) * k]) for i in range(n)]
+
+    def fixRecord(self, record):
+        if self._push_inputs() != 0:
+            raise RuntimeError("invalid parameters")
+        c = record.to_c()
+        shape = (C.c_int * 6)()
+        n = self._L.miqp_solver_fix_record(self._h, C.byref(c), None, 0, shape)
+        if n < 0:
+            raise RuntimeError("miqp_solver_fix_record refused the record (%d)" % n)
+        out = np.empty(n, dtype=np.int8)
+        if self._L.miqp_solver_fix_record(self._h, C.byref(c), out.ctypes.data_as(C.POINTER(C.c_byte)), n, shape) != n:
+            raise RuntimeError("miqp_solver_fix_record failed")
+        return out, tuple(shape)
+
+    def decodeProbe(self, records, big=False, walk=True, c2n=None):
+        if self._push_inputs() != 0:
+            raise RuntimeError("invalid parameters")
+        n = len(records)
+        keep = [r.to_c() for r in records]
+        ptrs = (C.POINTER(RawResultsC) * max(n, 1))(*[C.pointer(c) for c in keep])
+        stride = self._L.miqp_solver_decode_probe(self._h, ptrs, 0, None, int(bool(big)), int(bool(walk)), None, 0)
+        if stride < 0:
+            raise RuntimeError("miqp_solver_decode_probe refused the instance (%d)" % stride)
+        if n == 0:
+            return []
+        steps = records[0].dims[1]
+        m = None
+        if c2n is not None:
+            m = np.ascontiguousarray(c2n, dtype=np.int8)
+            cars = records[0].dims[0]
+            if m.shape != (n, cars * (cars - 1) // 2 * steps * 4):
+                raise ValueError("c2n: %r, expected (%d, pairs * steps * 4)" % (m.shape, n))
+        out = np.zeros(n * stride, dtype=np.uint8)
+        rc = self._L.miqp_solver_decode_probe(self._h, ptrs, n, m.ctypes.data_as(C.POINTER(C.c_byte)) if m is not None else None, int(bool(big)), int(bool(walk)),
+                                              out.ctypes.data_as(C.POINTER(C.c_ubyte)), out.size)
+        if rc != stride:
+            raise RuntimeError("miqp_solver_decode_probe failed (%d)" % rc)
+        G = 320 if big else 128
+        fields = [("head", "<i4", 4), ("sstart", "<i4", steps + 2), ("bkey", "<u8", steps * 32), ("cand", "<u2", G), ("gmeta", "<u4", G * 4),
+                  ("gcoef", "<f8", 432 if G == 128 else G * 7 // 2), ("grhs", "<f8", G)]
+        res = []
+        for k in range(n):
+            raw = out[k * stride:(k + 1) * stride]
+            d, o = {"raw": raw}, 0
+            for name, dt, cnt in fields:
+                d[name] = raw[o:o + cnt * np.dtype(dt).itemsize].view(dt)
+                o += (cnt * np.dtype(dt).itemsize + 7) & ~7
+            assert o == stride, (o, stride)
+            res.append(d)
+        return res
 
     def solveFixedBatch(self, records):
         if self._push_inputs() != 0:
```

Measured after the change: 1059. -1.9%, worse.
